# BUTSpeechFIT/x-vector-kaldi-tf

Hardware: AMD Instinct MI355X
Metric: utterances/sec (= x-vectors/sec, 512-d) on synthetic 23-dim MFCC, T~U[200,400] (higher is better)
Workload: dtype f32 in/out, f32 accumulate; GEMM products as fp16 MFMA + 2^-11 x scaled bf8 MFMA of the cross terms (layers 1-4) and bf16x3 split MFMA (layer 0, FC)

## Files before the change

include/xvector_hip.h:

```cpp
#ifndef XVECTOR_HIP_H_
#define XVECTOR_HIP_H_

#include <stddef.h>
#include <stdint.h>

#ifdef __cplusplus
extern "C" {
#endif

#define XV_ACT_NONE 0
#define XV_ACT_RELU 1
#define XV_ACT_LRELU 2
#define XV_ACT_PRELU 3

#define XV_ERR_BAD_ARG (-1)
#define XV_ERR_UNSUPPORTED (-2)

int xv_version(void);
const char *xv_last_error(void);
#define XV_TUNE_TILE_ROWS 1
#define XV_TUNE_FIRST_TILES 2
#define XV_TUNE_FP32_GEMM 3
int xv_set_tuning(int key, int value);

int xv_pack_weights_f32(const float *w, int kred, int cout, float *wp, void *stream);

int xv_fold_bn_f32(const float *gamma, const float *beta, const float *mean, const float *var, float eps,
                   int c, float *scale, float *shift, void *stream);

int xv_fold_shift_taps_f32(const float *w, const float *shift, const float *bias, int K, int cin, int cout, float *tap_bias,
                           float *bias_full, void *stream);

int xv_tdnn_layer_f32(const float *x, int64_t R, int cin, int ldx, const float *wp, const float *bias,
                      const float *bn_scale, const float *bn_shift, int act_kind, const float *act_alpha,
                      int K, int dilation, int cout, const uint8_t *row_valid, float *y, int ldy,
                      float *y_preact, void *stream);

size_t xv_packed_weights_rows_f32_floats(int K, int cin, int ldx, int cout);
int xv_pack_weights_rows_f32(const float *w, int K, int cin, int ldx, int cout, float *wp, void *stream);
int xv_tdnn_layer_rows_f32(const float *x, int64_t R, int cin, int ldx, const float *wp, const float *bias, const float *bn_scale,
                           const float *bn_shift, int act_kind, const float *act_alpha, int K, int cout, const uint8_t *row_valid,
                           float *y, int ldy, void *stream);

int xv_toom_supported(int K, int dilation, int cin, int cout);
size_t xv_packed_weights_toom_f32_floats(int K, int cin, int cout);
int xv_pack_weights_toom_f32(const float *w, int K, int cin, int cout, float *wp, void *stream);
int xv_tdnn_layer_toom_f32(const float *x, int64_t R, int cin, int ldx, const float *wp, const float *bias, const float *bn_scale,
                           const float *bn_shift, int act_kind, const float *act_alpha, int K, int cout, const uint8_t *row_valid,
                           float *y, int ldy, void *stream);
int xv_tdnn_layer_toom_dilated_f32(const float *x, int64_t R, int cin, int ldx, const float *wp, const float *bias, const float *bn_scale,
                                   const float *bn_shift, int act_kind, const float *act_alpha, int K, int dilation, int cout,
                                   const uint8_t *row_valid, float *y, int ldy, void *stream);

#define XV_FMT_F32 0
#define XV_FMT_SPLIT 1
#define XV_SPLIT_PAD_BEFORE 8
#define XV_SPLIT_PAD_AFTER 264
size_t xv_packed_weights_bf16x3_bytes(int K, int cin, int cout);
int xv_pack_weights_bf16x3(const float *w, int K, int cin, int cout, void *wt, void *stream);
int xv_pack_weights_bf16x3_many(int n, const float *const *w, const int32_t *K, const int32_t *cin, const int32_t *cin_pad,
                                const int32_t *cout, void *const *wt_fwd, void *const *wt_bwd, void *stream);
size_t xv_split_row_bytes(int channels);
int xv_split_encode_f32(const float *x, int64_t R, int c, int ldx, void *xs, void *stream);
int xv_split_decode_f32(const void *xs, int64_t R, int c, float *x, int ldx, void *stream);
int xv_tdnn_layer_bf16x3(const void *x, int x_format, int64_t R, int cin, int ldx, const void *wt, const float *bias,
                         const float *bn_scale, const float *bn_shift, int act_kind, const float *act_alpha, int K, int dilation,
                         int cout, const uint8_t *row_valid, void *y, int y_format, int ldy, float *y_preact, int ldpre,
                         void *stream);
int xv_tdnn_layer_bf16x3_sums(const void *x, int x_format, int64_t R, int cin, int ldx, const void *wt, const float *bias,
                              const float *bn_scale, const float *bn_shift, int act_kind, const float *act_alpha, int K,
                              int dilation, int cout, const uint8_t *row_valid, float *y, int ldy, const float *sum_r,
                              int ld_sum_r, void *workspace, void *stream);
int xv_tdnn_layer_bf16x3_moments(const void *x, int x_format, int64_t R, int cin, int ldx, const void *wt, const float *bias,
                                 const float *bn_scale, const float *bn_shift, int act_kind, const float *act_alpha, int K,
                                 int dilation, int cout, const uint8_t *row_valid, float *y, int ldy, float *y_preact, int ldpre,
                                 void *workspace, void *stream);
size_t xv_block_stats_bytes(int64_t R, int cout);
int xv_tdnn_layer_pool_bf16x3(const void *x, int x_format, int64_t R, int cin, int ldx, const void *wt, const float *bias,
                              const float *bn_scale, const float *bn_shift, int act_kind, const float *act_alpha, int K,
                              int dilation, int cout, const uint8_t *row_valid, float *block_stats, void *stream);
int xv_stats_pool_blocks_f32(const float *block_stats, int c, const int32_t *row_start, const int32_t *row_len, int nchunks,
                             float eps, float *out, void *stream);
int xv_tdnn_layer_pool_f32(const float *x, int64_t R, int cin, int ldx, const float *wp, const float *bias, const float *bn_scale,
                           const float *bn_shift, int act_kind, const float *act_alpha, int K, int dilation, int cout,
                           const uint8_t *row_valid, float *block_stats, void *stream);

size_t xv_packed_first_bf16x3_bytes(int K, int cin, int cout);
int xv_pack_first_bf16x3(const float *w, int K, int cin, int cout, void *wt, void *stream);
int xv_tdnn_first_bf16x3(const float *x, int64_t R, int cin, int ldx, const void *wt, const float *bias, const float *bn_scale,
                         const float *bn_shift, int act_kind, const float *act_alpha, int K, int dilation, int cout,
                         const uint8_t *row_valid, void *y, void *stream);

size_t xv_packed_pair_bf16x3_bytes(int cin, int cmid, int cout);
int xv_pack_pair_bf16x3(const float *w1, const float *w2, int cin, int cmid, int cout, void *wt, void *stream);
int xv_tdnn_pair_pool_bf16x3(const void *x, int64_t R, int cin, int cmid, int cout, const void *wt, const float *bias1,
                             const float *bn_scale1, const float *bn_shift1, const float *act_alpha1, const float *bias2,
                             const float *bn_scale2, const float *bn_shift2, const float *act_alpha2, int act_kind,
                             const uint8_t *row_valid, float *block_stats, void *stream);

#define XV_FMT_SPLIT8 2
size_t xv_packed_weights_f16bf8_bytes(int K, int cin, int cout);
int xv_pack_weights_f16bf8(const float *w, int K, int cin, int cout, void *wt, void *stream);
int xv_split8_encode_f32(const float *x, int64_t R, int c, int ldx, void *xs, int32_t *status, void *stream);
int xv_split8_decode_f32(const void *xs, int64_t R, int c, float *x, int ldx, void *stream);
int xv_tdnn_layer_f16bf8(const void *x, int64_t R, int cin, const void *wt, const float *bias, const float *bn_scale,
                         const float *bn_shift, int act_kind, const float *act_alpha, int K, int dilation, int cout,
                         const uint8_t *row_valid, const float *tap_bias, void *y, int y_format, int ldy, int32_t *status,
                         void *stream);
int xv_tdnn_layer_pool_f16bf8(const void *x, int64_t R, int cin, const void *wt, const float *bias, const float *bn_scale,
                              const float *bn_shift, int act_kind, const float *act_alpha, int K, int dilation, int cout,
                              const uint8_t *row_valid, const float *tap_bias, float *block_stats, void *stream);
int xv_tdnn_first_f16bf8(const float *x, int64_t R, int cin, int ldx, const void *wt, const float *bias, const float *bn_scale,
                         const float *bn_shift, int act_kind, const float *act_alpha, int K, int dilation, int cout,
                         const uint8_t *row_valid, void *y, int32_t *status, void *stream);

size_t xv_packed_pair_f16bf8_bytes(int cin, int cmid, int cout);
int xv_pack_pair_f16bf8(const float *w1, const float *w2, int cin, int cmid, int cout, void *wt, void *stream);
int xv_tdnn_pair_pool_f16bf8(const void *x, int64_t R, int cin, int cmid, int cout, const void *wt, const float *bias1,
                             const float *bn_scale1, const float *bn_shift1, const float *act_alpha1, const float *bias2,
                             const float *bn_scale2, const float *bn_shift2, const float *act_alpha2, int act_kind,
                             const uint8_t *row_valid, float *block_stats, int32_t *status, void *stream);

size_t xv_packed_pair_f16mx6_bytes(int cin, int cmid, int cout);
int xv_pack_pair_f16mx6(const float *w1, const float *w2, int cin, int cmid, int cout, void *wt, void *stream);
int xv_tdnn_pair_pool_f16mx6(const void *x, int64_t R, int cin, int cmid, int cout, const void *wt, const float *bias1,
                             const float *bn_scale1, const float *bn_shift1, const float *act_alpha1, const float *bias2,
                             const float *bn_scale2, const float *bn_shift2, const float *act_alpha2, int act_kind,
                             const uint8_t *row_valid, float *block_stats, int32_t *status, void *stream);

#define XV_FMT_SPLIT6 3
size_t xv_packed_weights_f16mx6_bytes(int K, int cin, int cout);
int xv_pack_weights_f16mx6(const float *w, int K, int cin, int cout, void *wt, void *stream);
int xv_split6_encode_f32(const float *x, int64_t R, int c, int ldx, void *xs, int32_t *status, void *stream);
int xv_split6_decode_f32(const void *xs, int64_t R, int c, float *x, float *cq, int ldx, void *stream);
int xv_tdnn_layer_f16mx6(const void *x, int64_t R, int cin, const void *wt, const float *bias, const float *bn_scale,
                         const float *bn_shift, int act_kind, const float *act_alpha, int K, int dilation, int cout,
                         const uint8_t *row_valid, const float *tap_bias, void *y, int y_format, int ldy, int32_t *status,
                         void *stream);

int xv_fc_bf16x3(const float *x, int nrows, int in_dim, const void *wt, const float *bias, const float *bn_scale,
                 const float *bn_shift, int act_kind, const float *act_alpha, int out_dim, float *y, float *y_preact, void *stream);

size_t xv_stats_pool_workspace_bytes(int c, int nchunks, int max_len, int split_rows);
int xv_stats_pool_f32(const float *h, int64_t ldh, int c, const int32_t *row_start, const int32_t *row_len,
                      int nchunks, int max_len, int split_rows, float eps, float *out, void *workspace,
                      void *stream);

int xv_fc_f32(const float *x, int nrows, int in_dim, const float *wp, const float *bias, const float *bn_scale,
              const float *bn_shift, int act_kind, const float *act_alpha, int out_dim, float *y,
              float *y_preact, void *stream);

size_t xv_fc_splitk_workspace_bytes(int nrows, int in_dim, int out_dim);
int xv_fc_splitk_f32(const float *x, int nrows, int in_dim, const float *wp, const float *bias, const float *bn_scale,
                     const float *bn_shift, int act_kind, const float *act_alpha, int out_dim, float *y, float *y_preact, void *workspace,
                     void *stream);

int xv_chunk_average_f32(const float *e, const int32_t *seg_start, const int32_t *chunk_len, int nutts, int dim,
                         float *out, void *stream);


int xv_chunk_moments_f32(const float *h, int64_t ldh, int c, const int32_t *row_start, const int32_t *row_len, int nchunks,
                         int max_len, int split_rows, float *out, void *workspace, void *stream);
int xv_merge_moments_f32(const float *chunk_mean_var, const int32_t *row_len, int nchunks, int c, float *mean, float *var,
                         void *stream);
int xv_rows_affine_f32(const float *x, int ldx, int64_t R, int c, const float *scale, const float *shift,
                       const uint8_t *row_valid, float *y, int ldy, void *stream);
int xv_rows_affine_split_f32(const float *x, int ldx, int64_t R, int c, const float *scale, const float *shift,
                             const uint8_t *row_valid, float *y, int ldy, void *y_split, void *stream);
size_t xv_wgrad_workspace_bytes(int64_t R, int cin, int cout, int K);
int xv_wgrad_f32(const float *x, int ldx, const float *dz, int lddz, int64_t R, int cin, int cout, int K, int dilation,
                 float *dw, void *workspace, void *stream);
int xv_wgrad_bf16x3(const float *x, int ldx, const float *dz, int lddz, int64_t R, int cin, int cout, int K, int dilation,
                    float *dw, void *workspace, void *stream);
size_t xv_wgrad_bias_workspace_bytes(int64_t R, int cin, int cout, int K);
int xv_wgrad_bias_bf16x3(const float *x, int ldx, const float *dz, int lddz, int64_t R, int cin, int cout, int K, int dilation,
                         float *dw, float *db, void *workspace, void *stream);
size_t xv_col_sums_workspace_bytes(int64_t R, int c);
int xv_col_sums_f32(const float *a, int lda, const float *b, int ldb, int64_t R, int c, float *sum_a, float *sum_ab,
                    void *workspace, void *stream);
int xv_bn_act_backward_f32(const float *dh, const float *r, int ld, int64_t R, int c, const float *sum_dh,
                           const float *sum_dh_r, const float *mean, const float *var, const float *gamma, float eps,
                           float n_frames, int act_kind, float act_alpha, const uint8_t *row_valid, float *dgamma,
                           float *dbeta, float *coef_ws, float *dz, void *stream);
int xv_bn_act_backward_split_f32(const float *dh, const float *r, int ld, int64_t R, int c, const float *sum_dh,
                                 const float *sum_dh_r, const float *mean, const float *var, const float *gamma, float eps,
                                 float n_frames, int act_kind, float act_alpha, const uint8_t *row_valid, float *dgamma,
                                 float *dbeta, float *coef_ws, float *dz, void *dz_split, void *stream);
int xv_bn_act_backward_parts_f32(const float *dh, const float *r, int ld, int64_t R, int c, const void *sums_workspace,
                                 const float *mean, const float *var, const float *gamma, float eps, float n_frames,
                                 int act_kind, float act_alpha, const uint8_t *row_valid, float *dgamma, float *dbeta,
                                 float *coef_ws, float *dz, void *dz_split, void *stream);
int xv_bn_moments_fold_f32(const void *sums_workspace, int64_t R, int c, float n_frames, const float *gamma, const float *beta,
                           float eps, float *mean, float *var, float *scale, float *shift, void *stream);
int xv_col_sums_merge_f32(const void *sums_workspace, int64_t R, int c, float *sum_a, float *sum_ab, void *stream);
int xv_pool_bn_act_backward_f32(const float *h, const float *r, int ld, int c, const int32_t *row_start, const int32_t *row_len,
                                int nchunks, int64_t R, const float *pooled, const float *dpooled, const float *chunk_moments,
                                const float *mean, const float *var, const float *gamma, float eps, float n_frames,
                                int act_kind, float act_alpha, float *dgamma, float *dbeta, float *coef_ws, float *dz,
                                void *dz_split, void *stream);
int xv_bn_small_forward_f32(const float *x, int ldx, int nrows, int c, const float *gamma, const float *beta, float eps, float *mean,
                            float *var, float *y, int ldy, void *stream);
int xv_bn_small_backward_f32(const float *dh, const float *r, int ld, int nrows, int c, const float *mean, const float *var,
                             const float *gamma, float eps, int act_kind, float act_alpha, float *dgamma, float *dbeta, float *dz,
                             void *stream);
int xv_pool_backward_f32(const float *h, int ldh, int c, const int32_t *row_start, const int32_t *row_len, int nchunks,
                         int64_t R, const float *pooled, const float *dpooled, float *dh, void *stream);
int xv_softmax_ce_f32(const float *logits, const int32_t *labels, int nrows, int nclasses, float *loss_acc, float *row_ws,
                      float *dlogits, void *stream);
int xv_adam_f32(float *param, const float *grad, float *m, float *v, int64_t n, float lr_t, float beta1, float beta2, float eps,
                void *stream);
int xv_axpy_f32(float *y, const float *x, float a, int64_t n, void *stream);
size_t xv_sumsq_workspace_bytes(int64_t n);
int xv_sumsq_f32(const float *x, int64_t n, float *out, void *workspace, void *stream);
int xv_dropout_f32(float *x, int ldx, int64_t R, int c, uint64_t seed, float keep_prob, void *stream);
int xv_minibatch_layout(int B, int T, int gap, int64_t rows, int32_t *row_start, int32_t *row_len, uint8_t *row_valid, void *stream);
int xv_pack_minibatch_f32(const void *src, int src_is_f16, int B, int T, int F, int gap, int in_dim, float *dst, int64_t rows,
                          void *stream);

int xv_prelu_backward_f32(float *dr, float *z, int ld, int64_t R, int c, const float *alpha, void *stream);

int xv_ema_f32(float *moving, const float *batch, int n, float decay, void *stream);

int xv_l2_normalize_rows_f32(const float *x, int ldx, int nrows, int c, float *y, int ldy, float *norm, void *stream);
int xv_l2_normalize_backward_f32(const float *dy, const float *y, const float *norm, int nrows, int c, float *dx, void *stream);
int xv_am_margin_f32(float *cosines, const int32_t *labels, int nrows, int nclasses, float scale, float margin, void *stream);

int xv_attention_scores_f32(const float *u, int64_t ldu, int64_t R, int c, const float *v, float *scores, float *nonlin,
                            int64_t ldn, void *stream);
int xv_attention_softmax_f32(const float *scores, const int32_t *row_start, const int32_t *row_len, int nchunks, float *att,
                             void *stream);
size_t xv_attention_pool_workspace_bytes(int c, int nchunks, int max_len, int split_rows);
int xv_attention_pool_f32(const float *h, int64_t ldh, int c, const float *att, const int32_t *row_start, const int32_t *row_len,
                          int nchunks, int max_len, int split_rows, float eps, float *out, void *workspace, void *stream);
int xv_attention_pool_backward_f32(const float *h, int64_t ldh, int c, const float *att, const int32_t *row_start,
                                   const int32_t *row_len, int nchunks, int max_len, const float *pooled, const float *dpooled,
                                   float *dh, int64_t lddh, float *datt, void *stream);
int xv_attention_softmax_backward_f32(const float *att, const float *datt, const int32_t *row_start, const int32_t *row_len,
                                      int nchunks, float *dscores, void *stream);
int xv_attention_scores_backward_f32(float *nonlin, int64_t ldn, const float *dscores, const float *v, int64_t R, int c, float *du,
                                     int64_t lddu, void *stream);

int xv_cmn_sliding_scatter_f32(const float *x, int ldx, int feat_dim, const int32_t *utt_start, const int32_t *utt_len,
                               int n_utts, int max_len, int cmn_window, int center, int min_window, const int32_t *dst_row,
                               float *y, int ldy, void *stream);

#define XV_BACKEND_KSTEP 8
#define XV_SIDE_PLAIN 0
#define XV_SIDE_ENROL 1
#define XV_SIDE_TEST 2
#define XV_SIDE_COSINE 3
int xv_backend_prepare_f32(const float *x, int64_t ldx, int n_rows, int dim_in, const int32_t *num_utts, const float *mean,
                           const float *lda, int64_t ld_lda, const float *lda_offset, int dim, int length_norm,
                           const float *plda_transform, const float *plda_mean, const float *plda_psi, int side, float *out,
                           int64_t ldo, float *r, void *stream);
int xv_score_matrix_f32(const float *e, const float *t, int64_t ldk, int kpad, int n_enrol, int n_test, const float *r,
                        float *scores, int64_t ld_scores, void *stream);
int xv_score_blocks_f32(const float *e, const float *t, int64_t ldk, int kpad, int n_rows, const float *r, const int32_t *grp_row0,
                        const int64_t *grp_score0, int n_groups, int max_n, float *scores, int64_t scores_elems, int32_t *status,
                        void *stream);
int xv_score_pairs_f32(const float *e, const float *t, int64_t ldk, int kpad, const int32_t *e_idx, const int32_t *t_idx,
                       int64_t n_trials, const float *r, float *scores, void *stream);
int xv_topk_row_stats_f32(const float *scores, int64_t ld, int n_rows, int n_cols, int top_n, float *mean, float *std,
                          void *stream);

#define XV_MOMENT_SLAB 2048
int xv_moment_stats_f64(const float *x, int64_t ldx, int64_t n_rows, int dim, double *sum, double *outer, int64_t ld_outer,
                        void *workspace, size_t workspace_bytes, void *stream);
size_t xv_moment_stats_workspace_bytes(int64_t n_rows, int dim);

#define XV_AHC_MAX_N 32768
int xv_ahc_average_f64(const float *scores, int64_t ld, int n, double threshold, int min_clusters, int32_t *merge_a,
                       int32_t *merge_b, double *merge_score, int32_t *n_merges, int32_t *labels, void *workspace,
                       size_t workspace_bytes, void *stream);
size_t xv_ahc_average_workspace_bytes(int n);

#define XV_AHC_BATCH_MAX_N 4096
int xv_ahc_average_batch_f64(const float *scores, int64_t scores_elems, const int32_t *grp_row0, const int64_t *grp_score0,
                             const int64_t *grp_ws0, const double *threshold, const int32_t *min_clusters, int n_groups, int max_n,
                             int n_rows, int32_t *merge_a, int32_t *merge_b, double *merge_score, int32_t *n_merges, int32_t *labels,
                             int32_t *status, void *workspace, size_t workspace_bytes, void *stream);
size_t xv_ahc_average_batch_workspace_bytes(int n);

#define XV_PCA_MAX_DIM 128
#define XV_PCA_MAX_SWEEPS 30
int xv_pca_plda_groups_f64(const float *y, int64_t ldy, int n_rows, const int32_t *grp_row0, int n_groups, int dim,
                           double target_energy, const double *mean, const double *within, const double *between,
                           const double *transform, const double *psi, int32_t *grp_dim, int32_t *grp_info, double *eigvals,
                           double *pca, double *grp_psi, double *grp_map, double *grp_off, int32_t *status, void *workspace,
                           size_t workspace_bytes, void *stream);
size_t xv_pca_plda_groups_workspace_bytes(int n_groups, int dim);
int xv_backend_prepare_groups_f32(const float *y, int64_t ldy, int n_rows, const int32_t *grp_row0, int n_groups, int max_n, int dim,
// ... 118 lines not shown
```

x-vector-kaldi-tf_amd/csrc/xv_first.hip:

```cpp
#include "xv_device.h"
#include "xv_split8.h"

namespace {

std::atomic<int> g_first_tiles{0};

constexpr int FR_WAVES = 8;
constexpr int FR_TILES = 3;
constexpr int FR_NKS = 4;
constexpr int FR_PASS_COLS = 128;
constexpr int FR_W_BYTES = (FR_PASS_COLS / 16) * FR_NKS * 2048;
constexpr int FR_P_OFF = 2 * FR_W_BYTES;
constexpr int FR_MAX_COUT = 512;
constexpr size_t FR_LDS_BYTES = FR_P_OFF + 4 * FR_MAX_COUT * 4;
constexpr int SROW = 128;
static_assert(FR_TILES == 3, "tdnn_first_kernel dispatches first_block<.., 1 | 2 | 3>");

struct FirstParams {
    const float *x;
    long R;
    int ldx, kc;
    int K, dil, cout;
    const uint8_t *wt;
    const float *bias, *scale, *shift, *alpha;
    int act;
    const uint8_t *valid;
    uint8_t *y;
    int ychunks;
    long row_base, rows_here;
    long n_tiles;
    int tpw;
    int *status;
};

template <int MODE>
__device__ __forceinline__ float first_act(float z, float a)
{
    if constexpr (MODE == 2) return __builtin_bit_cast(float, max(__builtin_bit_cast(int, z), 0));
    return MODE == 1 ? fmaxf(a * z, z) : MODE == 2 ? fmaxf(z, 0.f) : fmaxf(z, 0.f) + a * fminf(z, 0.f);
}

template <int HALF>
__device__ __forceinline__ float sub_f16_half(float c, int hpair)
{
    float r;
    if constexpr (HALF == 0)
        asm("v_fma_mix_f32 %0, %1, -1.0, %2 op_sel:[0,0,0] op_sel_hi:[1,0,0]" : "=v"(r) : "v"(hpair), "v"(c));
    else
        asm("v_fma_mix_f32 %0, %1, -1.0, %2 op_sel:[1,0,0] op_sel_hi:[1,0,0]" : "=v"(r) : "v"(hpair), "v"(c));
    return r;
}

constexpr int FR_STORE_AUX = 2;

template <int MODE, bool Y8, int NT, bool MASK, bool CLAMP>
__device__ __forceinline__ void first_block(const bf16x8 (&xh)[FR_TILES][FR_NKS], const bf16x8 (&xl)[FR_TILES][FR_NKS],
                                            const bf16x8 (&wh0)[FR_NKS], const bf16x8 (&wl0)[FR_NKS], const bf16x8 (&wh1)[FR_NKS],
                                            const bf16x8 (&wl1)[FR_NKS], const f32x4 b0, const f32x4 b1, const f32x4 s0, const f32x4 s1,
                                            const f32x4 o0, const f32x4 o1, const f32x4 a0, const f32x4 a1, const int (&keepm)[FR_TILES],
                                            const unsigned (&hioff)[FR_TILES], const int slab_off, const __amdgpu_buffer_rsrc_t yrs,
                                            float &amax)
{
    f32x4 m0[NT], m1[NT];
    auto mfma_tile = [&](int j) {
        m0[j] = b0; m1[j] = b1;
#pragma unroll
        for (int u = 0; u < FR_NKS; ++u) {
            m0[j] = __builtin_amdgcn_mfma_f32_16x16x32_bf16(wl0[u], xh[j][u], m0[j], 0, 0, 0);
            m1[j] = __builtin_amdgcn_mfma_f32_16x16x32_bf16(wl1[u], xh[j][u], m1[j], 0, 0, 0);
            m0[j] = __builtin_amdgcn_mfma_f32_16x16x32_bf16(wh0[u], xl[j][u], m0[j], 0, 0, 0);
            m1[j] = __builtin_amdgcn_mfma_f32_16x16x32_bf16(wh1[u], xl[j][u], m1[j], 0, 0, 0);
            m0[j] = __builtin_amdgcn_mfma_f32_16x16x32_bf16(wh0[u], xh[j][u], m0[j], 0, 0, 0);
            m1[j] = __builtin_amdgcn_mfma_f32_16x16x32_bf16(wh1[u], xh[j][u], m1[j], 0, 0, 0);
        }
    };
    auto epilogue = [&](int j) {
        const f32x4 z0 = m0[j], z1 = m1[j];
        float v[8];
#pragma unroll
        for (int e = 0; e < 4; e += 2) {
            const f32x2 r0 = {first_act<MODE>(z0[e], a0[e]), first_act<MODE>(z0[e + 1], a0[e + 1])};
            const f32x2 r1 = {first_act<MODE>(z1[e], a1[e]), first_act<MODE>(z1[e + 1], a1[e + 1])};
            const f32x2 y0 = __builtin_elementwise_fma(r0, (f32x2){s0[e], s0[e + 1]}, (f32x2){o0[e], o0[e + 1]});
            const f32x2 y1 = __builtin_elementwise_fma(r1, (f32x2){s1[e], s1[e + 1]}, (f32x2){o1[e], o1[e + 1]});
            v[e] = y0[0]; v[e + 1] = y0[1]; v[4 + e] = y1[0]; v[5 + e] = y1[1];
        }
        if constexpr (Y8) {
            typedef _Float16 f16x2 __attribute__((ext_vector_type(2)));
            typedef short s16x2 __attribute__((ext_vector_type(2)));
            xv_i32x4 vh, vx;
            float lo[8];
#pragma unroll
            for (int i = 0; i < 8; i += 2) {
                amax = fmaxf(amax, fmaxf(fabsf(v[i]), fabsf(v[i + 1])));
                float ca = v[i], cb = v[i + 1];
                if constexpr (CLAMP) {
                    ca = __builtin_amdgcn_fmed3f(ca, -XV_SPLIT8_MAX, XV_SPLIT8_MAX);
                    cb = __builtin_amdgcn_fmed3f(cb, -XV_SPLIT8_MAX, XV_SPLIT8_MAX);
                }
                if constexpr (MASK) {
                    ca = __builtin_bit_cast(float, __builtin_bit_cast(int, ca) & keepm[j]);
                    cb = __builtin_bit_cast(float, __builtin_bit_cast(int, cb) & keepm[j]);
                }
                const f16x2 h = {(_Float16)ca, (_Float16)cb};
                vh[i >> 1] = __builtin_bit_cast(int, h);
                lo[i] = sub_f16_half<0>(ca, vh[i >> 1]);
                lo[i + 1] = sub_f16_half<1>(cb, vh[i >> 1]);
                v[i] = ca; v[i + 1] = cb;
            }
            constexpr float inv = 1.f / XV_SPLIT8_LO_SCALE;
            s16x2 t0 = {0, 0}, t1 = {0, 0};
            t0 = __builtin_amdgcn_cvt_scalef32_pk_bf8_f32(t0, lo[0], lo[1], inv, false);
            t0 = __builtin_amdgcn_cvt_scalef32_pk_bf8_f32(t0, lo[2], lo[3], inv, true);
            t1 = __builtin_amdgcn_cvt_scalef32_pk_bf8_f32(t1, lo[4], lo[5], inv, false);
            t1 = __builtin_amdgcn_cvt_scalef32_pk_bf8_f32(t1, lo[6], lo[7], inv, true);
            int h0 = __builtin_amdgcn_cvt_pk_bf8_f32(v[0], v[1], 0, false);
            h0 = __builtin_amdgcn_cvt_pk_bf8_f32(v[2], v[3], h0, true);
            int h1 = __builtin_amdgcn_cvt_pk_bf8_f32(v[4], v[5], 0, false);
            h1 = __builtin_amdgcn_cvt_pk_bf8_f32(v[6], v[7], h1, true);
            vx = (xv_i32x4){__builtin_bit_cast(int, t0), __builtin_bit_cast(int, t1), h0, h1};
            __builtin_amdgcn_raw_buffer_store_b128(vh, yrs, hioff[j], slab_off, FR_STORE_AUX);
            __builtin_amdgcn_raw_buffer_store_b128(vx, yrs, hioff[j] ^ 64u, slab_off, FR_STORE_AUX);
        } else {
            bf16x8 vh, vl;
#pragma unroll
            for (int e = 0; e < 8; ++e) {
                const float m = MASK ? __builtin_bit_cast(float, __builtin_bit_cast(int, v[e]) & keepm[j]) : v[e];
                const __bf16 h = (__bf16)m;
                vh[e] = h;
                vl[e] = (__bf16)(m - (float)h);
            }
            __builtin_amdgcn_raw_buffer_store_b128(__builtin_bit_cast(xv_i32x4, vh), yrs, hioff[j], slab_off, FR_STORE_AUX);
            __builtin_amdgcn_raw_buffer_store_b128(__builtin_bit_cast(xv_i32x4, vl), yrs, hioff[j] ^ 64u, slab_off, FR_STORE_AUX);
        }
    };
    mfma_tile(0);
    __builtin_amdgcn_sched_barrier(0);
#pragma unroll
    for (int j = 1; j < NT; ++j) {
        mfma_tile(j);
        epilogue(j - 1);
        __builtin_amdgcn_sched_barrier(0);
    }
    epilogue(NT - 1);
    __builtin_amdgcn_sched_barrier(0);
}

template <int MODE, bool Y8>
__global__ __launch_bounds__(FR_WAVES * 64) void tdnn_first_kernel(const FirstParams p)
{
    extern __shared__ __attribute__((aligned(16))) char lds[];
    const int tid = threadIdx.x;
    const int lane = tid & 63;
    const int wave = __builtin_amdgcn_readfirstlane(tid >> 6);
    const int G = lane >> 4, f = lane & 15;
    const long tile0 = ((long)blockIdx.x * FR_WAVES + wave) * p.tpw;
    const int left = ((p.K - 1) * p.dil) >> 1;
    const int n_pass = (p.cout + FR_PASS_COLS - 1) / FR_PASS_COLS;
    const int n_groups = (p.tpw + FR_TILES - 1) / FR_TILES;
    const int steps = n_groups * n_pass;
    const unsigned yrow = (unsigned)p.ychunks * SROW;
    const __amdgpu_buffer_rsrc_t yrs = __builtin_amdgcn_make_buffer_rsrc(p.y + (size_t)p.row_base * yrow, 0, (int)(unsigned)(p.rows_here * yrow), XV_RSRC_FLAGS);

    auto fetch_weights = [&](int ps, int buf) {
        const int pieces = (min(FR_PASS_COLS, p.cout - ps * FR_PASS_COLS) >> 5) * 2 * FR_NKS * 2;
        const uint8_t *src = p.wt + (size_t)ps * FR_W_BYTES + lane * 16;
        char *dst = lds + buf * FR_W_BYTES;
        for (int pc = wave; pc < pieces; pc += FR_WAVES) XV_GLDS16_OFF(src + (size_t)pc * 1024, dst + pc * 1024, 0);
    };
    const int rot = (int)(blockIdx.x % (unsigned)n_pass);
    fetch_weights(rot, 0);
    {
        float *P = reinterpret_cast<float *>(lds + FR_P_OFF);
        for (int c = tid; c < p.cout; c += FR_WAVES * 64) {
            P[c] = p.bias ? p.bias[c] : 0.f;
            P[FR_MAX_COUT + c] = p.scale ? p.scale[c] : 1.f;
            P[2 * FR_MAX_COUT + c] = p.shift ? p.shift[c] : 0.f;
            P[3 * FR_MAX_COUT + c] = p.act == XV_ACT_NONE ? 1.f : p.act == XV_ACT_LRELU ? p.alpha[0] : p.act == XV_ACT_PRELU ? p.alpha[c] : 0.f;
        }
    }
    const f32x4 *P4 = reinterpret_cast<const f32x4 *>(lds + FR_P_OFF);

    bf16x8 xh[FR_TILES][FR_NKS], xl[FR_TILES][FR_NKS];
    int keepm[FR_TILES];
    unsigned hioff[FR_TILES];
    bool group_masked = false, clamping = false;
    int n_live = 0;
    float amax = 0.f;
    int pass = rot, group = 0, in_group = 0;
    int stores_behind_fetch = -1;

    for (int s = 0; s < steps; ++s) {
        if (in_group == 0) {
            const long gtile = tile0 + (long)group * FR_TILES;
            const long lrow0 = gtile * 16;
            n_live = 0;
#pragma unroll
            for (int j = 0; j < FR_TILES; ++j) {
                const bool ex = group * FR_TILES + j < p.tpw && gtile + j < p.n_tiles;
                n_live += ex ? 1 : 0;
                const long lrow = lrow0 + 16 * j + f, row = p.row_base + lrow;
                const bool in = ex && lrow < p.rows_here;
                keepm[j] = (in && (!p.valid || p.valid[row])) ? -1 : 0;
                hioff[j] = in ? (unsigned)lrow * yrow + (unsigned)((G ^ ((int)(row >> 1) & 7)) << 4) : 0x80000000u;
            }
#pragma unroll
            for (int u = 0; u < FR_NKS; ++u) {
                const int k = 32 * u + 8 * G;
                const int tap = k / p.kc;
                const bool live = tap < p.K;
                const int tap_off = tap * p.dil - left;
                const int c0 = k - tap * p.kc;
#pragma unroll
                for (int j = 0; j < FR_TILES; ++j) {
                    const long r = p.row_base + lrow0 + 16 * j + f + tap_off;
                    f32x4 a = {0.f, 0.f, 0.f, 0.f}, b = a;
                    if (live && j < n_live && r >= 0 && r < p.R) {
                        const float *src = p.x + (size_t)r * p.ldx + c0;
                        a = *reinterpret_cast<const f32x4 *>(src);
                        b = *reinterpret_cast<const f32x4 *>(src + 4);
                    }
#pragma unroll
                    for (int e = 0; e < 4; ++e) {
                        const __bf16 ha = (__bf16)a[e], hb = (__bf16)b[e];
                        xh[j][u][e] = ha; xh[j][u][4 + e] = hb;
                        xl[j][u][e] = (__bf16)(a[e] - (float)ha); xl[j][u][4 + e] = (__bf16)(b[e] - (float)hb);
                    }
                }
            }
            group_masked = __builtin_amdgcn_ballot_w64(keepm[0] == 0 || keepm[1] == 0 || keepm[2] == 0) != 0;
            stores_behind_fetch = -1;
        }
        if (stores_behind_fetch == 2 * 4 * FR_TILES) asm volatile("s_waitcnt vmcnt(24)" ::: "memory");
        else if (stores_behind_fetch == 2 * 4 * (FR_TILES - 1)) asm volatile("s_waitcnt vmcnt(16)" ::: "memory");
        else asm volatile("s_waitcnt vmcnt(0)" ::: "memory");
        __syncthreads();
        const int n_pairs = min(FR_PASS_COLS, p.cout - pass * FR_PASS_COLS) >> 5;
        if (s + 1 < steps) fetch_weights(pass + 1 == n_pass ? 0 : pass + 1, (s + 1) & 1);
        stores_behind_fetch = 0;
        const char *wbuf = lds + (s & 1) * FR_W_BYTES + lane * 16;

        if (n_live > 0) {
            for (int t = 0; t < n_pairs; ++t) {
                const int tp = (t + wave) % n_pairs;
                bf16x8 wh0[FR_NKS], wl0[FR_NKS], wh1[FR_NKS], wl1[FR_NKS];
                const char *w0 = wbuf + (size_t)(tp * 2) * (FR_NKS * 2048);
#pragma unroll
                for (int u = 0; u < FR_NKS; ++u) {
                    wh0[u] = *reinterpret_cast<const bf16x8 *>(w0 + u * 2048);
                    wl0[u] = *reinterpret_cast<const bf16x8 *>(w0 + u * 2048 + 1024);
                    wh1[u] = *reinterpret_cast<const bf16x8 *>(w0 + FR_NKS * 2048 + u * 2048);
                    wl1[u] = *reinterpret_cast<const bf16x8 *>(w0 + FR_NKS * 2048 + u * 2048 + 1024);
                }
                const int cb = pass * FR_PASS_COLS + tp * 32 + 8 * G;
                const int c4 = cb >> 2;
                const f32x4 b0 = P4[c4], b1 = P4[c4 + 1], s0 = P4[FR_MAX_COUT / 4 + c4], s1 = P4[FR_MAX_COUT / 4 + c4 + 1],
                            o0 = P4[2 * FR_MAX_COUT / 4 + c4], o1 = P4[2 * FR_MAX_COUT / 4 + c4 + 1];
                f32x4 a0 = {0.f, 0.f, 0.f, 0.f}, a1 = a0;
                if constexpr (MODE != 2) { a0 = P4[3 * FR_MAX_COUT / 4 + c4]; a1 = P4[3 * FR_MAX_COUT / 4 + c4 + 1]; }
                const int slab_off = (pass * (FR_PASS_COLS / 32) + tp) * SROW;
                auto run = [&](auto nt, auto mask, auto clamp) {
                    first_block<MODE, Y8, decltype(nt)::value, decltype(mask)::value, decltype(clamp)::value>(
                        xh, xl, wh0, wl0, wh1, wl1, b0, b1, s0, s1, o0, o1, a0, a1, keepm, hioff, slab_off, yrs, amax);
                };
                auto run_nt = [&](auto mask, auto clamp) {
                    if (n_live == 3) run(std::integral_constant<int, 3>{}, mask, clamp);
                    else if (n_live == 2) run(std::integral_constant<int, 2>{}, mask, clamp);
                    else run(std::integral_constant<int, 1>{}, mask, clamp);
                };
                if (Y8 && clamping) run_nt(std::true_type{}, std::true_type{});
                else {
                    if (group_masked) run_nt(std::true_type{}, std::false_type{});
                    else run_nt(std::false_type{}, std::false_type{});
                    if (Y8 && __builtin_amdgcn_ballot_w64(!(amax <= XV_SPLIT8_MAX)) != 0) {
                        clamping = true;
                        run_nt(std::true_type{}, std::true_type{});
                        stores_behind_fetch = -1000;
                    }
                }
                stores_behind_fetch += 2 * n_live;
            }
        }
        if (++pass == n_pass) pass = 0;
        if (++in_group == n_pass) { in_group = 0; ++group; }
    }
    if constexpr (Y8)
        if (amax > XV_SPLIT8_MAX && p.status) atomicOr(p.status, 1);
}

__global__ void pack_first_kernel(const float *__restrict__ w, int K, int cin, int kc, int cout, uint8_t *__restrict__ wt, size_t total)
{
    const size_t i = (size_t)blockIdx.x * blockDim.x + threadIdx.x;
    if (i >= total) return;
    const int e = (int)(i & 7);
    const int lane = (int)((i >> 3) & 63);
    constexpr int TILES = FR_PASS_COLS / 16;
    const int u = (int)((i >> 9) & 3);
    const int tile = (int)((i >> 11) & (TILES - 1));
    const int pass = (int)(i / (size_t)(512 * FR_NKS * TILES));
    const int k = 32 * u + 8 * (lane >> 4) + e;
    const int tap = k / kc, c = k - tap * kc;
    const int i_row = lane & 15;
    const int col = pass * FR_PASS_COLS + 32 * (tile >> 1) + 8 * (i_row >> 2) + 4 * (tile & 1) + (i_row & 3);
    const float x = (tap < K && c < cin && col < cout) ? w[((size_t)tap * cin + c) * cout + col] : 0.f;
    const __bf16 hi = (__bf16)x;
    const __bf16 lo = (__bf16)(x - (float)hi);
    uint8_t *t = wt + (size_t)pass * FR_W_BYTES + (size_t)(tile * FR_NKS + u) * 2048 + lane * 16 + e * 2;
    *reinterpret_cast<uint16_t *>(t) = __builtin_bit_cast(uint16_t, hi);
    *reinterpret_cast<uint16_t *>(t + 1024) = __builtin_bit_cast(uint16_t, lo);
}

bool first_shape_ok(int K, int cin, int cout)
{
    const int kc = (cin + 7) / 8 * 8;
    return K > 0 && (K & 1) && cin > 0 && K * kc <= 32 * FR_NKS && cout > 0 && (cout & 31) == 0 && cout <= FR_MAX_COUT;
}

}

extern "C" {

void xv_internal_first_tiles(int tiles) { g_first_tiles.store(tiles, std::memory_order_relaxed); }

size_t xv_packed_first_bf16x3_bytes(int K, int cin, int cout)
{
    if (!first_shape_ok(K, cin, cout)) return 0;
    return (size_t)((cout + FR_PASS_COLS - 1) / FR_PASS_COLS) * FR_W_BYTES;
}

int xv_pack_first_bf16x3(const float *w, int K, int cin, int cout, void *wt, void *stream)
{
    if (!w || !wt) return fail(XV_ERR_BAD_ARG, "pack_first_bf16x3: NULL pointer");
    if (!first_shape_ok(K, cin, cout))
        return fail(XV_ERR_UNSUPPORTED, "pack_first_bf16x3: needs K odd, K*ceil8(cin) <= 128, cout % 32 == 0, cout <= 512");
    const size_t total = xv_packed_first_bf16x3_bytes(K, cin, cout) / 4;
    hipLaunchKernelGGL(pack_first_kernel, dim3((unsigned)((total + 255) / 256)), dim3(256), 0, (hipStream_t)stream, w, K, cin,
                       (cin + 7) / 8 * 8, cout, (uint8_t *)wt, total);
    return launch_status();
}

static int first_launch(const float *x, int64_t R, int cin, int ldx, const void *wt, const float *bias, const float *bn_scale,
                        const float *bn_shift, int act_kind, const float *act_alpha, int K, int dilation, int cout,
                        const uint8_t *row_valid, void *y, bool y8, int32_t *status, void *stream)
{
    if (R <= 0) return 0;
    if (!x || !wt || !y) return fail(XV_ERR_BAD_ARG, "tdnn_first: NULL pointer");
    if (act_kind < XV_ACT_NONE || act_kind > XV_ACT_PRELU) return fail(XV_ERR_BAD_ARG, "tdnn_first: unknown act_kind");
    if ((act_kind == XV_ACT_LRELU || act_kind == XV_ACT_PRELU) && !act_alpha) return fail(XV_ERR_BAD_ARG, "tdnn_first: act_alpha is NULL");
    const int kc = (cin + 7) / 8 * 8;
    if (!first_shape_ok(K, cin, cout) || dilation <= 0 || (K - 1) * dilation > 8)
        return fail(XV_ERR_UNSUPPORTED, "tdnn_first: needs K odd, K*ceil8(cin) <= 128, (K-1)*dilation <= 8, cout % 32 == 0, cout <= 512");
    if (ldx < kc || (ldx & 7) || (((uintptr_t)x) & 31))
        return fail(XV_ERR_UNSUPPORTED, "tdnn_first: rows must hold ceil8(cin) floats (padding columns zero), ldx % 8 == 0, x 32-byte aligned");
    if ((((uintptr_t)wt) | ((uintptr_t)y)) & 15) return fail(XV_ERR_BAD_ARG, "tdnn_first: wt and y must be 16-byte aligned");
    FirstParams p{};
    p.x = x; p.R = (long)R; p.ldx = ldx; p.kc = kc; p.K = K; p.dil = dilation; p.cout = cout; p.wt = (const uint8_t *)wt;
    p.bias = bias; p.scale = bn_scale; p.shift = bn_shift; p.alpha = act_alpha; p.act = act_kind; p.valid = row_valid;
    p.y = (uint8_t *)y; p.ychunks = cout / 32; p.status = (int *)status;
    typedef void (*kern_t)(const FirstParams);
    const kern_t kerns[6] = {tdnn_first_kernel<0, false>, tdnn_first_kernel<1, false>, tdnn_first_kernel<2, false>,
                             tdnn_first_kernel<0, true>,  tdnn_first_kernel<1, true>,  tdnn_first_kernel<2, true>};
    static std::atomic<unsigned long long> lds_done{0};
    if (const int rc = opt_in_dynamic_lds(lds_done, kerns, FR_LDS_BYTES)) return rc;
    const int mode = act_kind == XV_ACT_LRELU ? 1 : act_kind == XV_ACT_RELU ? 2 : 0;
    static std::atomic<int> n_cu{0};
    int cus = n_cu.load(std::memory_order_relaxed);
    if (cus <= 0) {
        int dev = 0;
        (void)hipGetDevice(&dev);
        if (hipDeviceGetAttribute(&cus, hipDeviceAttributeMultiprocessorCount, dev) != hipSuccess || cus <= 0) cus = 256;
        n_cu.store(cus, std::memory_order_relaxed);
    }
    const int forced = g_first_tiles.load(std::memory_order_relaxed);
    const long waves = (long)cus * FR_WAVES;
    constexpr long MAX_ROWS = 1L << 19;
    for (long r0 = 0; r0 < p.R; r0 += MAX_ROWS) {
        p.row_base = r0;
        p.rows_here = p.R - r0 < MAX_ROWS ? p.R - r0 : MAX_ROWS;
        p.n_tiles = (p.rows_here + 15) / 16;
        p.tpw = forced > 0 ? forced : (int)((p.n_tiles + waves - 1) / waves);
        const long per_wg = (long)p.tpw * FR_WAVES;
        hipLaunchKernelGGL(kerns[mode + (y8 ? 3 : 0)], dim3((unsigned)((p.n_tiles + per_wg - 1) / per_wg)), dim3(FR_WAVES * 64), FR_LDS_BYTES,
                           (hipStream_t)stream, p);
    }
    return launch_status();
}

int xv_tdnn_first_bf16x3(const float *x, int64_t R, int cin, int ldx, const void *wt, const float *bias, const float *bn_scale,
                         const float *bn_shift, int act_kind, const float *act_alpha, int K, int dilation, int cout,
                         const uint8_t *row_valid, void *y, void *stream)
{
    return first_launch(x, R, cin, ldx, wt, bias, bn_scale, bn_shift, act_kind, act_alpha, K, dilation, cout, row_valid, y, false,
                        nullptr, stream);
}

int xv_tdnn_first_f16bf8(const float *x, int64_t R, int cin, int ldx, const void *wt, const float *bias, const float *bn_scale,
                         const float *bn_shift, int act_kind, const float *act_alpha, int K, int dilation, int cout,
                         const uint8_t *row_valid, void *y, int32_t *status, void *stream)
{
    return first_launch(x, R, cin, ldx, wt, bias, bn_scale, bn_shift, act_kind, act_alpha, K, dilation, cout, row_valid, y, true,
                        status, stream);
}

}
```

x-vector-kaldi-tf_amd/csrc/xv_kernels.hip:

```cpp
#include "xv_device.h"

namespace {

thread_local char g_err[256] = "";

constexpr int BM = 128;
constexpr int BN = 128;
constexpr int BK = 32;
constexpr int LDS_LD = 36;
constexpr int A_ROWS = BM + MAX_SPAN;
constexpr int NT = 256;

struct GemmParams {
    const float *x;
    long R;
    int cin, ldx;
    const float *wp;
    int kred;
    const float *bias, *scale, *shift;
    int act;
    const float *alpha;
    int K, dil, cout;
    const uint8_t *valid;
    float *y;
// ... 610 lines not shown
        X.b0 = *reinterpret_cast<const f32x4 *>(glds + bb);
        X.b1 = *reinterpret_cast<const f32x4 *>(glds + bb + 32 * G_SROW);
    };
    auto mma = [&](const Fr &X) {
#pragma unroll
        for (int j = 0; j < 4; ++j) {
            acc00 = __builtin_amdgcn_mfma_f32_32x32x2f32(X.a0[j], X.b0[j], acc00, 0, 0, 0);
            acc01 = __builtin_amdgcn_mfma_f32_32x32x2f32(X.a0[j], X.b1[j], acc01, 0, 0, 0);
            acc10 = __builtin_amdgcn_mfma_f32_32x32x2f32(X.a1[j], X.b0[j], acc10, 0, 0, 0);
            acc11 = __builtin_amdgcn_mfma_f32_32x32x2f32(X.a1[j], X.b1[j], acc11, 0, 0, 0);
        }
    };
    auto pin = [&]() {
#pragma unroll
        for (int i = 0; i < 4; ++i) {
            __builtin_amdgcn_sched_group_barrier(0x008, 1, 0);
            __builtin_amdgcn_sched_group_barrier(0x100, 1, 0);
        }
        __builtin_amdgcn_sched_group_barrier(0x008, 12, 0);
        __builtin_amdgcn_sched_barrier(0);
    };
    Fr F, G;
    load(F, 0, 0);
    for (int s = 0; s < n_stages; ++s) {
        load(G, s & 1, 1);
        mma(F);
        pin();
        asm volatile("s_waitcnt vmcnt(0) lgkmcnt(0)" ::: "memory");
        __builtin_amdgcn_s_barrier();
        dma(s + 2, s & 1);
        __builtin_amdgcn_sched_barrier(0);
        load(F, (s + 1) & 1, 0);
        mma(G);
        pin();
    }
    asm volatile("s_waitcnt vmcnt(0)" ::: "memory");
    __syncthreads();
    switch (p.act) {
    case XV_ACT_RELU: k1_epilogue<XV_ACT_RELU>(p, glds, Ms, m0, n0, wr, wc, tid, acc00, acc01, acc10, acc11); break;
    case XV_ACT_LRELU: k1_epilogue<XV_ACT_LRELU>(p, glds, Ms, m0, n0, wr, wc, tid, acc00, acc01, acc10, acc11); break;
    case XV_ACT_PRELU: k1_epilogue<XV_ACT_PRELU>(p, glds, Ms, m0, n0, wr, wc, tid, acc00, acc01, acc10, acc11); break;
    default: k1_epilogue<XV_ACT_NONE>(p, glds, Ms, m0, n0, wr, wc, tid, acc00, acc01, acc10, acc11); break;
    }
}

std::atomic<int> g_fp32_form{0};

int launch_gemm(const GemmParams &p0, hipStream_t st)
{
    GemmParams p = p0;
    if (p.R <= 0 || p.cout <= 0) return 0;
    if (p.cin <= 0 || p.K <= 0 || (p.K & 1) == 0 || p.dil <= 0) return fail(XV_ERR_BAD_ARG, "tdnn: K must be odd, dims > 0");
    if ((p.K - 1) * p.dil > MAX_SPAN) return fail(XV_ERR_UNSUPPORTED, "tdnn: (K-1)*dilation > 8 unsupported");
    if ((p.lead == 0 && p.ldx < p.cin) || p.ldy < p.cout) return fail(XV_ERR_BAD_ARG, "tdnn: leading dimension too small");
    if ((p.act == XV_ACT_LRELU || p.act == XV_ACT_PRELU) && !p.alpha) return fail(XV_ERR_BAD_ARG, "tdnn: act_alpha is NULL");
    p.kred = p.K * p.cin;
    p.n_nt = (p.cout + BN - 1) / BN;
    const bool small = ((p.R + BM - 1) / BM) * p.n_nt < 768;
    const int bmt = small ? 64 : BM;
    p.n_mt = (int)((p.R + bmt - 1) / bmt);
    const bool vec = (p.cin % 4 == 0) && (p.ldx % 4 == 0) && (((uintptr_t)p.x) % 16 == 0) && (((uintptr_t)p.wp) % 16 == 0);
    if (p.lead && (!vec || p.K != 1 || p.ypre)) return fail(XV_ERR_UNSUPPORTED, "tdnn_rows: needs 16-byte aligned rows of a multiple of 4 floats");
    const uintptr_t out_bits = (uintptr_t)p.y | (uintptr_t)p.ypre | (uintptr_t)p.bias | (uintptr_t)p.scale | (uintptr_t)p.shift |
                               (p.act == XV_ACT_PRELU ? (uintptr_t)p.alpha : 0);
    p.vec_out = (p.cout % 4 == 0) && (p.ldy % 4 == 0) && (out_bits % 16 == 0);
    if (p.blk && !p.vec_out) return fail(XV_ERR_UNSUPPORTED, "tdnn_pool: needs cout % 4 == 0 and 16-byte aligned per-column parameters");
    typedef void (*kern_t)(const GemmParams);
    const kern_t all[] = {tdnn_gemm_kernel<true, 128>, tdnn_gemm_kernel<false, 128>, tdnn_gemm_kernel<true, 64>,
                          tdnn_gemm_kernel<false, 64>};
    const kern_t dma_all[] = {tdnn_gemm_dma_kernel<1>, tdnn_gemm_dma_kernel<3>, tdnn_gemm_dma_kernel<5>, tdnn_gemm_dma_kernel<7>};
    typedef std::pair<kern_t, size_t> kern_lds;
    const kern_lds lds[] = {{all[0], GEMM_LDS_BYTES}, {all[1], GEMM_LDS_BYTES}, {all[2], GEMM_LDS_BYTES}, {all[3], GEMM_LDS_BYTES},
                            {dma_all[0], F_LDS_BYTES}, {dma_all[1], F_LDS_BYTES}, {dma_all[2], F_LDS_BYTES}, {dma_all[3], F_LDS_BYTES},
                            {tdnn_gemm_k1_kernel, G_LDS_BYTES}};
    static std::atomic<unsigned long long> lds_done{0};
    if (const int rc = opt_in_dynamic_lds(lds_done, lds, [](const kern_lds &kl) { return kl; })) return rc;
    const dim3 grid((unsigned)(p.n_mt * p.n_nt));
    const int form = g_fp32_form.load(std::memory_order_relaxed);
    const bool dma_on = form != 1;
    const bool k1_on = form == 0 || form == 3;
    const bool dma_ok = dma_on && !small && p.k_splits <= 1 && vec && p.vec_out && (p.cin % BK) == 0 && (p.K == 1 || p.K == 3 || p.K == 5 || p.K == 7) &&
                        (p.R + BM + MAX_SPAN) * (long)p.ldx * 4 < (1l << 31) && (long)(p.cout + BN) * p.kred * 4 < (1l << 31);
    if (dma_ok && k1_on && p.K == 1 && p.cin >= 2 * G_BK) {
        hipLaunchKernelGGL(tdnn_gemm_k1_kernel, grid, dim3(NT), G_LDS_BYTES, st, p);
        return launch_status("tdnn_gemm_k1_kernel launch");
    }
    if (dma_ok) {
        const kern_t dk = p.K == 1 ? tdnn_gemm_dma_kernel<1> : p.K == 3 ? tdnn_gemm_dma_kernel<3> : p.K == 5 ? tdnn_gemm_dma_kernel<5>
                                                                                                             : tdnn_gemm_dma_kernel<7>;
        hipLaunchKernelGGL(dk, grid, dim3(NT), F_LDS_BYTES, st, p);
        return launch_status("tdnn_gemm_dma_kernel launch");
    }
    if (p.k_splits > 1) {
        hipLaunchKernelGGL(all[(small ? 2 : 0) + (vec ? 0 : 1)], dim3((unsigned)(p.n_mt * p.n_nt * p.k_splits)), dim3(NT), GEMM_LDS_BYTES, st, p);
        return launch_status("tdnn_gemm_kernel (split-K) launch");
    }
    hipLaunchKernelGGL(all[(small ? 2 : 0) + (vec ? 0 : 1)], grid, dim3(NT), GEMM_LDS_BYTES, st, p);
    return launch_status("tdnn_gemm_kernel launch");
}

__global__ void pack_weights_kernel(const float *__restrict__ w, int kred, int cout, float *__restrict__ wp)
{
    const size_t i = (size_t)blockIdx.x * blockDim.x + threadIdx.x;
    if (i >= (size_t)kred * cout) return;
    const int n = (int)(i / kred), k = (int)(i - (size_t)n * kred);
    wp[i] = w[(size_t)k * cout + n];
}

__global__ void pack_weights_rows_kernel(const float *__restrict__ w, int K, int cin, int ldx, int cout, int kpad, float *__restrict__ wp)
{
    const size_t i = (size_t)blockIdx.x * blockDim.x + threadIdx.x;
    if (i >= (size_t)kpad * cout) return;
    const int o = (int)(i / kpad), col = (int)(i - (size_t)o * kpad);
    const int k = col / ldx, c = col - k * ldx;
    wp[i] = (k < K && c < cin) ? w[((size_t)k * cin + c) * cout + o] : 0.f;
}

__global__ void fold_bn_kernel(const float *gamma, const float *beta, const float *mean, const float *var, float eps,
                               int c, float *scale, float *shift)
{
#pragma clang fp contract(off)
    const int i = blockIdx.x * blockDim.x + threadIdx.x;
    if (i >= c) return;
    const float s = gamma[i] * (1.0f / sqrtf(var[i] + eps));
    float ms = mean[i] * s;
    asm volatile("" : "+v"(ms));
    scale[i] = s;
    shift[i] = beta[i] - ms;
}

__global__ void fold_shift_taps_kernel(const float *__restrict__ w, const float *__restrict__ shift, const float *__restrict__ bias,
                                       int K, int cin, int cout, float *__restrict__ tap, float *__restrict__ bias_full)
{
    const int o = blockIdx.x * blockDim.x + threadIdx.x;
    if (o >= cout) return;
    double total = bias ? (double)bias[o] : 0.0;
    for (int t = 0; t < K; ++t) {
        double acc = 0.0;
        for (int c = 0; c < cin; ++c) acc += (double)shift[c] * (double)w[((size_t)t * cin + c) * cout + o];
        if (tap) tap[(size_t)t * cout + o] = (float)acc;
        total += acc;
    }
    bias_full[o] = (float)total;
}

}

extern "C" {

void xv_internal_gemm3_tile_rows(int value);
void xv_internal_gemm8_tile_rows(int value);
void xv_internal_first_tiles(int tiles);

int xv_version(void) { return 42; }

int xv_set_tuning(int key, int value)
{
    switch (key) {
    case XV_TUNE_TILE_ROWS:
        if (value != 0 && value != 128 && value != 256 && value != 512 && value != 1024)
            return fail(XV_ERR_BAD_ARG, "xv_set_tuning: tile rows must be 0, 128, 256, 512 or 1024");
        xv_internal_gemm3_tile_rows(value >= 512 ? 256 : value);
        xv_internal_gemm8_tile_rows(value);
        return 0;
    case XV_TUNE_FIRST_TILES:
        if (value < 0 || value > 4096) return fail(XV_ERR_BAD_ARG, "xv_set_tuning: first-layer tiles per wave must be 0 .. 4096");
        xv_internal_first_tiles(value);
        return 0;
    case XV_TUNE_FP32_GEMM:
        if (value < 0 || value > 3) return fail(XV_ERR_BAD_ARG, "xv_set_tuning: fp32 GEMM form must be 0, 1, 2 or 3");
        g_fp32_form.store(value, std::memory_order_relaxed);
        return 0;
    default:
        return fail(XV_ERR_BAD_ARG, "xv_set_tuning: unknown key");
    }
}

const char *xv_last_error(void) { return g_err; }

int xv_pack_weights_f32(const float *w, int kred, int cout, float *wp, void *stream)
{
    if (!w || !wp || kred <= 0 || cout <= 0) return fail(XV_ERR_BAD_ARG, "pack_weights: bad argument");
    const size_t n = (size_t)kred * cout;
    hipLaunchKernelGGL(pack_weights_kernel, dim3((unsigned)((n + 255) / 256)), dim3(256), 0, (hipStream_t)stream, w, kred, cout, wp);
    return launch_status("pack_weights_kernel");
}

int xv_fold_bn_f32(const float *gamma, const float *beta, const float *mean, const float *var, float eps, int c,
                   float *scale, float *shift, void *stream)
{
    if (!gamma || !beta || !mean || !var || !scale || !shift || c <= 0) return fail(XV_ERR_BAD_ARG, "fold_bn: bad argument");
    hipLaunchKernelGGL(fold_bn_kernel, dim3((c + 255) / 256), dim3(256), 0, (hipStream_t)stream, gamma, beta, mean, var, eps, c, scale, shift);
    return launch_status("fold_bn_kernel");
}

int xv_fold_shift_taps_f32(const float *w, const float *shift, const float *bias, int K, int cin, int cout, float *tap_bias,
                           float *bias_full, void *stream)
{
    if (!w || !shift || !bias_full || K <= 0 || cin <= 0 || cout <= 0) return fail(XV_ERR_BAD_ARG, "fold_shift_taps: bad argument");
    hipLaunchKernelGGL(fold_shift_taps_kernel, dim3((cout + 63) / 64), dim3(64), 0, (hipStream_t)stream, w, shift, bias, K, cin, cout,
                       tap_bias, bias_full);
    return launch_status("fold_shift_taps_kernel");
}

int xv_tdnn_layer_f32(const float *x, int64_t R, int cin, int ldx, const float *wp, const float *bias,
                      const float *bn_scale, const float *bn_shift, int act_kind, const float *act_alpha, int K,
                      int dilation, int cout, const uint8_t *row_valid, float *y, int ldy, float *y_preact,
                      void *stream)
{
    if (!x || !wp || (!y && !y_preact)) return fail(XV_ERR_BAD_ARG, "tdnn: NULL pointer");
    if (act_kind < XV_ACT_NONE || act_kind > XV_ACT_PRELU) return fail(XV_ERR_BAD_ARG, "tdnn: unknown act_kind");
    GemmParams p{};
    p.x = x; p.R = (long)R; p.cin = cin; p.ldx = ldx; p.wp = wp;
    p.bias = bias; p.scale = bn_scale; p.shift = bn_shift; p.act = act_kind; p.alpha = act_alpha;
    p.K = K; p.dil = dilation; p.cout = cout; p.valid = row_valid; p.y = y; p.ldy = ldy; p.ypre = y_preact;
    return launch_gemm(p, (hipStream_t)stream);
}

size_t xv_packed_weights_rows_f32_floats(int K, int cin, int ldx, int cout)
{
    if (K <= 0 || (K & 1) == 0 || cin <= 0 || ldx < cin || (ldx & 3) || cout <= 0) return 0;
    return (size_t)cout * (((size_t)K * ldx + BK - 1) / BK * BK);
}

int xv_pack_weights_rows_f32(const float *w, int K, int cin, int ldx, int cout, float *wp, void *stream)
{
    const size_t n = xv_packed_weights_rows_f32_floats(K, cin, ldx, cout);
    if (!w || !wp || n == 0) return fail(XV_ERR_BAD_ARG, "pack_weights_rows: K odd, cin <= ldx, ldx % 4 == 0");
    hipLaunchKernelGGL(pack_weights_rows_kernel, dim3((unsigned)((n + 255) / 256)), dim3(256), 0, (hipStream_t)stream, w, K, cin, ldx, cout,
                       (int)(n / cout), wp);
    return launch_status("pack_weights_rows_kernel");
}

int xv_tdnn_layer_rows_f32(const float *x, int64_t R, int cin, int ldx, const float *wp, const float *bias, const float *bn_scale,
                           const float *bn_shift, int act_kind, const float *act_alpha, int K, int cout, const uint8_t *row_valid,
                           float *y, int ldy, void *stream)
{
    if (!x || !wp || !y) return fail(XV_ERR_BAD_ARG, "tdnn_rows: NULL pointer");
    if (act_kind < XV_ACT_NONE || act_kind > XV_ACT_PRELU) return fail(XV_ERR_BAD_ARG, "tdnn_rows: unknown act_kind");
    const size_t n = xv_packed_weights_rows_f32_floats(K, cin, ldx, cout);
    if (n == 0) return fail(XV_ERR_BAD_ARG, "tdnn_rows: K odd, cin <= ldx, ldx % 4 == 0");
    GemmParams p{};
    p.x = x; p.R = (long)R; p.cin = (int)(n / cout); p.ldx = ldx; p.wp = wp;
    p.bias = bias; p.scale = bn_scale; p.shift = bn_shift; p.act = act_kind; p.alpha = act_alpha;
    p.K = 1; p.dil = 1; p.cout = cout; p.valid = row_valid; p.y = y; p.ldy = ldy; p.lead = (K - 1) / 2;
    return launch_gemm(p, (hipStream_t)stream);
}

int xv_tdnn_layer_pool_f32(const float *x, int64_t R, int cin, int ldx, const float *wp, const float *bias, const float *bn_scale,
                           const float *bn_shift, int act_kind, const float *act_alpha, int K, int dilation, int cout,
                           const uint8_t *row_valid, float *block_stats, void *stream)
{
    if (!x || !wp || !block_stats) return fail(XV_ERR_BAD_ARG, "tdnn_pool: NULL pointer");
    if (act_kind < XV_ACT_NONE || act_kind > XV_ACT_PRELU) return fail(XV_ERR_BAD_ARG, "tdnn_pool: unknown act_kind");
    if (((uintptr_t)block_stats) & 15) return fail(XV_ERR_BAD_ARG, "tdnn_pool: block_stats must be 16-byte aligned");
    GemmParams p{};
    p.x = x; p.R = (long)R; p.cin = cin; p.ldx = ldx; p.wp = wp;
    p.bias = bias; p.scale = bn_scale; p.shift = bn_shift; p.act = act_kind; p.alpha = act_alpha;
    p.K = K; p.dil = dilation; p.cout = cout; p.valid = row_valid; p.ldy = cout; p.blk = block_stats;
    return launch_gemm(p, (hipStream_t)stream);
}

int xv_fc_f32(const float *x, int nrows, int in_dim, const float *wp, const float *bias, const float *bn_scale,
              const float *bn_shift, int act_kind, const float *act_alpha, int out_dim, float *y, float *y_preact,
              void *stream)
{
    return xv_tdnn_layer_f32(x, nrows, in_dim, in_dim, wp, bias, bn_scale, bn_shift, act_kind, act_alpha, 1, 1,
                             out_dim, nullptr, y, out_dim, y_preact, stream);
}

static int splitk_groups(int nrows, int in_dim, int out_dim)
{
    if (nrows <= 0 || nrows > 128 || in_dim < 16 * BK) return 1;
    const int chunks = (in_dim + BK - 1) / BK;
    const int tiles = ((nrows + 63) / 64) * ((out_dim + BN - 1) / BN);
    int per = (chunks * tiles + 255) / 256;
    if (per < 2) per = 2;
    return (chunks + per - 1) / per;
}

size_t xv_fc_splitk_workspace_bytes(int nrows, int in_dim, int out_dim)
{
    const int g = splitk_groups(nrows, in_dim, out_dim);
    return g > 1 ? (size_t)g * nrows * out_dim * sizeof(float) : 0;
}

int xv_fc_splitk_f32(const float *x, int nrows, int in_dim, const float *wp, const float *bias, const float *bn_scale,
                     const float *bn_shift, int act_kind, const float *act_alpha, int out_dim, float *y, float *y_preact, void *workspace,
                     void *stream)
{
    const int g = splitk_groups(nrows, in_dim, out_dim);
    if (g <= 1) return xv_fc_f32(x, nrows, in_dim, wp, bias, bn_scale, bn_shift, act_kind, act_alpha, out_dim, y, y_preact, stream);
    if (!x || !wp || (!y && !y_preact) || !workspace) return fail(XV_ERR_BAD_ARG, "fc_splitk: NULL pointer");
    if (act_kind < XV_ACT_NONE || act_kind > XV_ACT_PRELU) return fail(XV_ERR_BAD_ARG, "fc_splitk: unknown act_kind");
    if ((act_kind == XV_ACT_LRELU || act_kind == XV_ACT_PRELU) && !act_alpha) return fail(XV_ERR_BAD_ARG, "fc_splitk: act_alpha is NULL");
    GemmParams p{};
    p.x = x; p.R = nrows; p.cin = in_dim; p.ldx = in_dim; p.wp = wp;
    p.act = XV_ACT_NONE; p.K = 1; p.dil = 1; p.cout = out_dim; p.ldy = out_dim;
    p.ypre = (float *)workspace;
    p.k_splits = g; p.part = (float *)workspace; p.part_stride = (long)nrows * out_dim;
    int rc = launch_gemm(p, (hipStream_t)stream);
    if (rc) return rc;
    const size_t n = (size_t)nrows * out_dim;
    hipLaunchKernelGGL(splitk_reduce_kernel, dim3((unsigned)((n + 255) / 256)), dim3(256), 0, (hipStream_t)stream, (const float *)workspace,
                       (long)nrows * out_dim, g, nrows, out_dim, bias, bn_scale, bn_shift, act_kind, act_alpha, y, out_dim, y_preact, out_dim);
    return launch_status("splitk_reduce_kernel");
}
// ... 5 lines not shown
```

x-vector-kaldi-tf_amd/local/tf/models.py:

```python
import io
import os
import sys
import time

import numpy as np

_PKG_ROOT = os.path.dirname(os.path.dirname(os.path.dirname(os.path.abspath(__file__))))
if _PKG_ROOT not in sys.path:
    sys.path.insert(0, _PKG_ROOT)

import kaldi_io
from xvector_amd import engine, extract_stream, frontend, synthetic, topology, weights as wio

VAR2STD_EPSILON = topology.VAR2STD_EPSILON


def _device():
    dev = os.environ.get("XVECTOR_DEVICE")
    if dev:
        return dev
    return "cuda:%d" % int(os.environ.get("LOCAL_RANK", "0"))


class VectorCollector(object):
# ... 2 lines not shown
    def __init__(self):
        self.keys, self.blocks = [], []

    def write_vectors(self, keys, vecs):
        if len(keys):
            self.keys.extend(keys)
            self.blocks.append(np.asarray(vecs, dtype=np.float32).reshape(len(keys), -1))

    def write(self, data):
        raise IOError("the sharded extractor writes vectors, not bytes")

    def __enter__(self):
        return self

    def __exit__(self, *a):
        return False


def gather_shard_vectors(device_model, collector, shard_keys, rank, world):
    import torch
    from xvector_amd import dist as xdist, jobclock
    dim, dev = device_model.embed_dim, device_model.device
    mine = shard_keys[rank]
    block = np.zeros((len(mine), dim + 1), np.float32)
    if collector.keys:
        whole = len(collector.keys) == len(mine) and mine == collector.keys
        if whole:
            rows = slice(None)
        else:
            rows, j = np.empty(len(collector.keys), np.int64), 0
            for i, k in enumerate(mine):
                if j < len(rows) and collector.keys[j] == k:
                    rows[j] = i
                    j += 1
            if j != len(rows):
                raise RuntimeError("sharded extraction: emitted keys are not a subsequence of the shard's keys")
        block[rows, 0] = 1.0
        if whole and len(collector.blocks) == 1:
            block[:, 1:] = collector.blocks[0]
        else:
            block[rows, 1:] = np.concatenate(collector.blocks)
    xdist.wait_process_group()
    jobclock.mark("wait for the process group")
    import torch.distributed as dist
    host = dist.is_initialized() and dist.get_backend() == "gloo"
    blocks = xdist.gather_blocks(torch.from_numpy(block) if host else torch.from_numpy(block).to(dev), [len(k) for k in shard_keys], 0)
    jobclock.mark("gather")
    if rank != 0:
        return None
    out = []
    for r in range(world):
        got = blocks[r].cpu().numpy()
        out.append((shard_keys[r], got[:, 1:], got[:, 0] > 0.5))
    return out


_SELECTED = {}
_IDLE_MODELS = {}
_IDLE_KEEP = 1


def _checkpoint_identity(model_dir):
    ident = []
    for name in ("model.weights.npz", "model.index", "model.data-00000-of-00001"):
        path = os.path.join(model_dir, name)
        try:
            st = os.stat(path)
            ident.append((os.path.realpath(path), st.st_mtime_ns, st.st_size))
        except OSError:
            pass
    return (tuple(ident) or None,)


class _StepDone(object):

    def __init__(self, value):
        self._value = value

    def result(self):
        return self._value


class Model(object):

    window_frames = 1 << 21
    first_window_frames = 1 << 18
    arena_bytes = 64 << 20
    first_arena_bytes = 64 << 20
    map_input = os.environ.get("XVECTOR_MAP_INPUT", "1") != "0"
    arena_count = 5
    exchange_windows = int(os.environ.get("XVECTOR_EXCHANGE_WINDOWS", "0"))
    max_batch_rows = 262144

    def __init__(self):
        self.graph = None
        self.device_model = None
        self.num_classes = None

    @classmethod
    def class_topology(cls):
        return topology.get(cls.__name__)

    def build_model(self, num_classes, input_feature_dim, output_dir, logger=None):
        if logger is not None:
            logger.info("Start building the model ...")
        topo = self.class_topology()
        self.num_classes = num_classes
        seed = int(os.environ.get("XVECTOR_INIT_SEED", "0"))
        w = synthetic.reference_init(topo, input_feature_dim, num_classes, seed=seed)
        self.save_model(dict(weights=w, topology=topo, model_class=type(self).__name__,
                             num_classes=num_classes, feat_dim=input_feature_dim), output_dir, logger)
        if logger is not None:
            logger.info("Building finished.")

    @staticmethod
    def save_model(sess, output_dir, logger):
        if logger is not None:
            logger.info("Start saving graph ...")
        wio.save_model_dir(output_dir, sess["weights"], sess["topology"], sess["model_class"],
                           sess["num_classes"], sess["feat_dim"])
        if logger is not None:
            logger.info("Graph saved in path: %s" % os.path.join(output_dir, "model"))

    def load_model(self, sess, input_dir, logger):
        if logger is not None:
            logger.info("Start loading graph ...")
        from xvector_amd import jobclock
        w, meta = wio.load_model_dir(input_dir)
        jobclock.once("weights read")
        import torch
        jobclock.once("import torch")
        torch.cuda.init()
        jobclock.once("hip runtime up")
        if getattr(self, "prepin_staging", False):
            try:
                engine.prewarm_staging((int(w["frame_level_info_layer-0/w:0"].shape[1]) + 3) // 4 * 4, self.max_batch_rows)
            except Exception:
                pass
        self.meta = meta
        self.num_classes = meta["num_classes"]
        self.embedding_index = int(os.environ.get("XVECTOR_EMBEDDING_INDEX", "0"))
        self.precision = os.environ.get("XVECTOR_PRECISION", "f16bf8")
        key = _checkpoint_identity(input_dir) + (self.precision, self.embedding_index, _device(), engine.PROBE_LIMIT_F16BF8,
                                                 engine.PROBE_LIMIT_BF16X3, os.environ.get("XVECTOR_ACCURACY_PROBE", "1"))
        known = _SELECTED.get(key)
        idle = _IDLE_MODELS.get(key)
        self._model_key = None
        if known is not None and idle and getattr(self, "_may_borrow", False):
            self.device_model = idle.pop()
            self._model_key = key
        elif known is not None:
            self.device_model = engine.DeviceModel(w, meta["topology"], _device(), self.embedding_index, known["selected"],
                                                   fold_shift=False if known.get("fold_shift") is False else None,
                                                   layer_mx6=False if known.get("layer_mx6") is False else None)
            self.device_model.selection = dict(known, cached=True)
            self._model_key = key
        else:
            self.device_model = engine.select_model(w, meta["topology"], _device(), self.embedding_index, self.precision)
            if key[0] is not None:
                _SELECTED[key] = dict(getattr(self.device_model, "selection", None) or {})
                self._model_key = key
        sel = getattr(self.device_model, "selection", None) or {}
        if logger is not None:
            if sel.get("probed"):
                logger.info("GEMM arithmetic: %s (requested %s; accuracy probe: f16bf8 vs bf16x3 %.2e%s)" % (
                    sel["selected"], sel["requested"], sel["f16bf8_vs_bf16x3"],
                    ", bf16x3 vs fp32 %.2e" % sel["bf16x3_vs_fp32"] if "bf16x3_vs_fp32" in sel else ""))
            logger.info("Graph restored from path: %s" % input_dir)

    def create_one_hot_output_matrix(self, labels):
        one_hot = np.zeros((len(labels), self.num_classes), dtype=np.int32)
        one_hot[np.arange(len(labels)), np.asarray(labels, dtype=np.int64)] = 1
        return one_hot

    def print_models_params(self, input_dir, logger=None):
        w, meta = wio.load_model_dir(input_dir)
        print('\n\nThe components are:\n')
        for name in wio.expected_names(meta["topology"]):
            if name.rsplit('/', 1)[-1] not in ("mean:0", "variance:0"):
                print(name)
        print('\n')

    def get_models_weights(self, input_dir, logger=None):
        h5file = os.path.join(input_dir, 'model.h5')
        try:
            import h5py
        except ImportError:
            h5py = None
        if h5py is not None and os.path.exists(h5file):
            name2weights = {}

            def collect(name, node):
                if not isinstance(node, h5py.Group):
                    name2weights[name] = np.array(node[()])
            with h5py.File(h5file, 'r') as hf:
                hf.visititems(collect)
            return name2weights
        w, meta = wio.load_model_dir(input_dir)
        name2weights = {}
        for name in wio.expected_names(meta["topology"]):
            if name.rsplit('/', 1)[-1] not in ("mean:0", "variance:0"):
                name2weights[name] = np.array(w[name], dtype=np.float32)
        for name in wio.expected_names(meta["topology"]):
            if name not in name2weights:
                name2weights[name] = np.array(w[name], dtype=np.float32)
        for name, mat in name2weights.items():
            print('%s  shape: %s' % (name, str(mat.shape)))
        if h5py is not None:
            with h5py.File(h5file, 'w') as hf:
                for name, mat in name2weights.items():
                    hf.create_dataset(name, data=mat.astype(np.float32))
        elif logger is not None:
            logger.info("h5py is not installed: %s not written" % h5file)
        return name2weights

    def _trainer(self, input_dir, logger, first_batch=None):
        from xvector_amd import trainer
        if logger is not None:
            logger.info("Start loading graph ...")
        w, meta = wio.load_model_dir(input_dir)
        self.meta = meta
        self.num_classes = meta["num_classes"]
        precision = os.environ.get("XVECTOR_TRAIN_PRECISION", "auto")
        adam = wio.load_optimizer_state(input_dir)
        self.train_precision_auto = precision == "auto"
        kept = wio.load_train_verdict(input_dir) if precision == "auto" and first_batch is not None else None
        if kept is not None:
            self.train_precision_verdict = dict(kept, iterations_since_probe=int(kept.get("iterations_since_probe", 0)) + 1, reused=True)
            tr = trainer.Trainer(w, meta["topology"], _device(), adam, precision=kept["selected"])
            if logger is not None:
                logger.info("Training arithmetic: %s (verdict of %d iteration(s) ago, kept with the model)" % (
                    kept["selected"], self.train_precision_verdict["iterations_since_probe"]))
        elif precision == "auto" and first_batch is not None:
            tr, verdict = trainer.select_trainer(w, meta["topology"], _device(), adam, first_batch[0], first_batch[1], logger)
            self.train_precision_verdict = dict(verdict, iterations_since_probe=0)
        else:
            tr = trainer.Trainer(w, meta["topology"], _device(), adam, precision="fp32" if precision == "auto" else precision)
        if logger is not None:
            logger.info("Graph restored from path: %s" % input_dir)
        return tr

    @staticmethod
    def _next_batch(data_loader, index, logger, what, meter):
        import queue
        t0 = time.time()
        try:
            batch, labels = data_loader.pop()
        except queue.Empty:
            logger.warning('Timeout reach when reading %s %d' % (what, index))
            batch, labels = None, None
        else:
            if batch is None:
                logger.warning('batch_data is None for %s %d' % (what, index))
        meter.waited("disk", time.time() - t0)
        return batch, labels

    @staticmethod
    def _everyone_has(batch, device):
        import torch.distributed as dist
        have = batch is not None
        if not (dist.is_available() and dist.is_initialized() and dist.get_world_size() > 1):
            return have
        import torch
        on_gpu = dist.get_backend() == "nccl"
        flag = torch.tensor([1 if have else 0], dtype=torch.int32, device=device if on_gpu else "cpu")
        dist.all_reduce(flag, op=dist.ReduceOp.MIN)
        return bool(flag.item())

    def train_one_iteration(self, data_loader, args, logger):
        from xvector_amd import runstats
        keep_out = float(getattr(args, "dropout_proportion", 0.0) or 0.0)
        seed = int(getattr(args, "random_seed", 0) or 0)
        tr = None
        pending = None
        meter = runstats.Meter(planned=data_loader.count, report_every=args.print_interval)
        for index in range(data_loader.count):
            batch, labels = self._next_batch(data_loader, index, logger, 'the minibatch index', meter)
            stepped_now = self._everyone_has(batch, _device())
            if not stepped_now:
                if batch is not None:
                    logger.warning('minibatch index %d skipped: another rank of the group has no batch' % index)
            else:
                if tr is None:
                    tr = self._trainer(args.input_dir, logger, (batch, labels))
                t0 = time.time()
                launch = getattr(tr, "step_async", None)
                handle = launch(batch, labels, args.learning_rate, keep_out, seed) if launch is not None else \
                    _StepDone(tr.step(batch, labels, args.learning_rate, keep_out, seed))
                now = (index, batch.shape[0], batch.shape[1], handle)
                if pending is not None:
                    meter.stepped(pending[0], pending[1], pending[2], *self._finite(pending, tr, args.input_dir, logger))
                pending = now
                meter.waited("gpu", time.time() - t0)
            if pending is not None and (index == data_loader.count - 1 or meter.interval_due(index)):
                meter.stepped(pending[0], pending[1], pending[2], *self._finite(pending, tr, args.input_dir, logger))
                pending = None
            if not stepped_now:
                meter.skipped(index)
            line = meter.interval_line(index)
            if line:
                logger.info(line)
        for line in meter.training_summary():
            logger.info(line)
        if tr is None:
            tr = self._trainer(args.input_dir, logger)
        if getattr(args, "save_model", True):
            w, adam = tr.export()
# ... 215 lines not shown
```

x-vector-kaldi-tf_amd/xvector_amd/engine.py:

```python
import ctypes
import math
import os
import threading

import numpy as np

from . import hiplib
from . import topology as tp

_HOST = []


def _host_lib():
    if not _HOST:
        lib = None
        path = os.path.join(os.path.dirname(os.path.dirname(os.path.abspath(__file__))), "local", "tf", "libxvector_host.so")
        try:
            if os.environ.get("XVECTOR_NO_HOST_LIB") == "1":
                raise OSError("disabled")
            lib = ctypes.CDLL(path)
            lib.xv_pack_rows_f32.restype = ctypes.c_int
            lib.xv_pack_rows_f32.argtypes = [ctypes.c_void_p, ctypes.c_void_p, ctypes.c_void_p, ctypes.c_int, ctypes.c_int,
                                             ctypes.c_void_p, ctypes.c_int64, ctypes.c_int64, ctypes.c_void_p, ctypes.c_int]
            lib.xv_raw_row_plan.restype = ctypes.c_int
# ... 61 lines not shown
    valid = np.flatnonzero((T > 0) & (T >= min_chunk_size))
    order = valid[np.argsort(T[valid], kind="stable")]
    To = T[order]
    cs = To if chunk_size == -1 else np.where(To < chunk_size, To, chunk_size)
    nch = -(-To // np.maximum(cs, 1))
    last = To - (nch - 1) * cs
    kept = nch - (last < min_chunk_size)
    seg = np.zeros(len(order) + 1, np.int64)
    np.cumsum(kept, out=seg[1:])
    c_utt = np.repeat(order, kept)
    idx = np.arange(int(seg[-1]), dtype=np.int64) - np.repeat(seg[:-1], kept)
    csr = np.repeat(cs, kept)
    c_start = idx * csr
    c_len = np.where(idx == np.repeat(nch - 1, kept), np.repeat(last, kept), csr)
    return order, c_utt, c_start, c_len, seg


def plan_subsegments(num_rows, min_chunk_size, window, period):
    if not 1 <= period <= window:
        raise ValueError("sub-segments need 1 <= period <= window (period %d, window %d)" % (period, window))
    if num_rows == 0 or num_rows < min_chunk_size:
        return None
    plan = [(0, min(window, num_rows))]
    k = 1
    while (k - 1) * period + window < num_rows:
        length = min(window, num_rows - k * period)
        if length < min_chunk_size:
            break
        plan.append((k * period, length))
        k += 1
    return plan


def plan_subsegment_table(lengths, min_chunk_size, window, period):
    if not 1 <= period <= window:
        raise ValueError("sub-segments need 1 <= period <= window (period %d, window %d)" % (period, window))
    T = np.asarray(lengths, dtype=np.int64)
    valid = np.flatnonzero((T > 0) & (T >= min_chunk_size))
    order = valid[np.argsort(T[valid], kind="stable")]
    To = T[order]
    kmax = np.where(To > window, -(-(To - window) // period), 0)
    last = np.minimum(window, To - kmax * period)
    kept = kmax + 1 - ((kmax > 0) & (last < min_chunk_size))
    seg = np.zeros(len(order) + 1, np.int64)
    np.cumsum(kept, out=seg[1:])
    c_utt = np.repeat(order, kept)
    idx = np.arange(int(seg[-1]), dtype=np.int64) - np.repeat(seg[:-1], kept)
    c_start = idx * period
    c_len = np.where(idx == np.repeat(kmax, kept), np.repeat(last, kept), window)
    return order, c_utt, c_start, c_len, seg


def device_plan_table(utt_start, utt_len, order, c_len, seg_start):
    return np.stack([np.asarray(utt_start)[order], np.asarray(utt_len)[order], c_len[seg_start[:-1]], np.diff(seg_start),
                     seg_start[:-1]]).astype(np.int32)


class BatchLayout(object):

    def __init__(self, lengths, gap, align=1):
        lengths = np.asarray(lengths, dtype=np.int64)
        self.gap = int(gap)
        self.align = int(align)
        self.row_len = lengths.astype(np.int32)
        self.lead = int(slot_rows(0, self.gap, self.align))
        self.slots = slot_rows(lengths, self.gap, self.align)
        starts = np.empty(len(lengths), dtype=np.int64)
        if len(lengths):
            starts[0] = self.lead
            np.cumsum(self.slots[:-1], out=starts[1:])
            starts[1:] += self.lead
        self.row_start = starts.astype(np.int32)
        self.rows = int(self.lead + self.slots.sum())
        self.nchunks = len(lengths)
        self.max_len = int(lengths.max()) if len(lengths) else 0
        assert self.rows < 2 ** 31

    def row_valid(self, out=None):
        n = self.nchunks
        vals = np.zeros(2 * n + 1, dtype=np.uint8)
        vals[1::2] = 1
        reps = np.empty(2 * n + 1, dtype=np.int64)
        reps[0] = self.lead
        reps[1::2] = self.row_len
        reps[2::2] = self.slots - self.row_len
        m = np.repeat(vals, reps)
        if out is not None:
            out[:self.rows] = m
            return out[:self.rows]
        return m

    def pack(self, mats, out):
        if not mats:
            out[:self.rows] = 0
            return
        F = mats[0].shape[1]
        z = np.zeros((self.gap + self.align, F), dtype=out.dtype)
        parts = [z[:self.lead]] * (2 * len(mats) + 1)
        parts[1::2] = mats
        if self.align > 1:
            parts[2::2] = [z[:g] for g in (self.slots - self.row_len).tolist()]
        elif self.lead != self.gap:
            raise AssertionError
        np.concatenate(parts, axis=0, out=out[:self.rows, :F])


def shift_tap_table(w3d, shift):
    return np.einsum("c,kco->ko", np.asarray(shift, np.float64), np.asarray(w3d, np.float64))


def folded_row_bias(bias, taps, row_valid, dilation):
    taps = np.asarray(taps, np.float64)
    K = taps.shape[0]
    v = np.asarray(row_valid, np.float64).reshape(-1)
    R = v.shape[0]
    halo = (K - 1) // 2 * int(dilation)
    vp = np.concatenate([np.zeros(halo), v, np.zeros(halo)])
    out = np.tile(np.asarray(bias, np.float64), (R, 1))
    for t in range(K):
        out += vp[t * int(dilation): t * int(dilation) + R, None] * taps[t][None, :]
    return out


class _ColumnView(object):

    def __init__(self, weights, cols):
        self.weights, self.cols = weights, cols

    def __getitem__(self, name):
        return self.weights[name][self.cols]


class _Layer(dict):

    def __missing__(self, key):
        if key == "wp" and "_make_wp" in self:
            self["wp"] = dict.pop(self, "_make_wp")()
            return self["wp"]
        raise KeyError(key)

    def ep(self, act):
        return self["bias"], self["scale"], self["shift"], act, self["alpha"]

    @property
    def pp(self):
        return self["bias"], self["scale"], self["shift"], self["alpha"]


class DeviceModel(object):

    POOL_SPLIT_ROWS = 512

    def __init__(self, weights, topo, device="cuda:0", embedding_index=0, precision="bf16x3", fused_pool=None, pair_kernel=None,
                 first_kernel=None, fold_shift=None, layer_mx6=None):
        import torch
        hiplib.require_gpu()
        assert precision in ("fp32", "fp32tc", "bf16x3", "f16bf8")
        self.toom = precision == "fp32tc"
        self.requested_precision = precision
        if self.toom:
            precision = "fp32"
        self.f16bf8 = False
        if precision == "f16bf8":
            precision = "bf16x3"
            ks, ds = list(topo["kernel_sizes"]), list(topo["dilations"])
            w0 = weights["frame_level_info_layer-0/w:0"]
            self.f16bf8 = (not tp.is_attention(topo) and fused_pool in (None, True) and len(ks) >= 3 and (ks[0] - 1) * ds[0] <= 8 and
                           all(hiplib.f16bf8_supported(k, d) for k, d in zip(ks[1:], ds[1:])))
        self.precision = precision
        self._weights = weights if self.f16bf8 else None
        self._fallback = None
        self.attention = tp.is_attention(topo)
        can_fuse = not self.attention and (precision == "bf16x3" or int(topo["layer_sizes"][-1]) % 4 == 0)
        self.fused_pool = can_fuse if fused_pool is None else bool(fused_pool)
        assert not (self.fused_pool and precision == "fp32" and int(topo["layer_sizes"][-1]) % 4), "fused fp32 pooling needs Cout % 4 == 0"
        assert not (self.fused_pool and self.attention), "the fused epilogue computes plain statistics, not attention-weighted ones"
        self.align = hiplib.POOL_BLOCK_ROWS if self.fused_pool else (2 if self.toom else 1)
        self.torch = torch
        self.device = torch.device(device)
        self.topo = topo
        self.embedding_index = int(embedding_index)
        self.gap = tp.max_halo(topo)
        self.act = tp.ACT_CODES[topo.get("activation", "relu")]
        self.feat_dim = int(weights["frame_level_info_layer-0/w:0"].shape[1])
        self.in_dim = (self.feat_dim + 3) // 4 * 4
        self.layers = []
        self._uploaded = {}
        with torch.cuda.device(self.device):
            for i, (k, d) in enumerate(zip(topo["kernel_sizes"], topo["dilations"])):
                sc = "frame_level_info_layer-%d" % i
                w = weights[sc + "/w:0"]
                assert w.shape[0] == k, "kernel size mismatch in %s" % sc
                if i == 0 and self.in_dim != self.feat_dim:
                    wpad = np.zeros((k, self.in_dim, w.shape[2]), np.float32)
                    wpad[:, :self.feat_dim] = w
                    w = wpad
                last = i == len(topo["kernel_sizes"]) - 1
                self.layers.append(self._prep(weights, sc, w, k, d, defer_wp=self.f16bf8, toom_ok=not (last and self.fused_pool)))
                if isinstance(self.layers[-1].get("wp"), hiplib.PackedToom) and d > 1:
                    self.align = math.lcm(self.align, 2 * int(d))
            if self.attention:
                A = self.layers[-1]["cout"] // 2
                self.att_dim = A
                aw = weights["attention/w:0"]
                assert aw.shape == (A, A), "attention/w:0 must be [%d, %d]" % (A, A)
                self.att = dict(K=1, dil=1, cin=A, cout=A, bias=self._dev(weights["attention/b:0"]),
                                v=self._dev(weights["attention/v:0"]))
                if precision == "bf16x3":
                    self.att["wp"] = hiplib.pack_weights_bf16x3(self._dev(aw[None, :, :]))
                    sc = "frame_level_info_layer-%d" % (len(self.layers) - 1)
                    k, d = topo["kernel_sizes"][-1], topo["dilations"][-1]
                    self.last_halves = [self._prep(weights, sc, weights[sc + "/w:0"], k, d, cols=slice(a, a + A)) for a in (0, A)]
                else:
                    self.att["wp"] = hiplib.pack_weights(self._dev(aw))
            self.first = None
            L0 = self.layers[0]
            if (first_kernel is None or first_kernel) and precision == "bf16x3" and len(self.layers) > 1 and \
                    self.in_dim % 8 == 0 and hiplib.first_supported(L0["K"], self.in_dim, L0["cout"]) and (L0["K"] - 1) * L0["dil"] <= 8:
                w0 = weights["frame_level_info_layer-0/w:0"]
                wpad = np.zeros((L0["K"], self.in_dim, w0.shape[2]), np.float32)
                wpad[:, :self.feat_dim] = w0
                self.first = hiplib.pack_first_bf16x3(self._dev(wpad))
            assert not (first_kernel and self.first is None), "first_kernel=True but the topology / precision does not allow it"
            self.pair = self.pair8 = self.pair_mx6 = None
            if (pair_kernel is None or pair_kernel) and self.fused_pool and precision == "bf16x3" and len(self.layers) >= 3:
                La, Lb = self.layers[-2], self.layers[-1]
                if La["K"] == 1 and Lb["K"] == 1 and hiplib.pair_supported(La["cin"], La["cout"], Lb["cout"]):
                    n = len(self.layers)
                    wa = self._wdev(weights, "frame_level_info_layer-%d/w:0" % (n - 2))[0]
                    wb = self._wdev(weights, "frame_level_info_layer-%d/w:0" % (n - 1))[0]
                    self.pair = hiplib.pack_pair_bf16x3(wa, wb)
                    if self.f16bf8 and hiplib.pair8_supported(La["cin"], La["cout"], Lb["cout"]):
                        self.pair8 = hiplib.pack_pair_f16bf8(wa, wb)
                        if hiplib.pair_mx6_supported(La["cin"], La["cout"], Lb["cout"]):
                            self.pair_mx6 = hiplib.pack_pair_f16mx6(wa, wb)
            assert not (pair_kernel and self.pair is None), "pair_kernel=True but the topology / precision does not allow it"
            if self.f16bf8:
                if self.first is None:
                    self.layers[0]["wp"]
                n = len(self.layers)
                for i in range(1, n - 2 if self.pair is not None else n):
                    sc = "frame_level_info_layer-%d" % i
                    self.layers[i]["wp8"] = hiplib.pack_weights_f16bf8(self._wdev(weights, sc + "/w:0"))
                self.status = torch.zeros(1, dtype=torch.int32, device=self.device)
            self.mx6_layers = set()
            if self.f16bf8 and (layer_mx6 is None or layer_mx6):
                def takes(j):
                    Lj = self.layers[j]
                    return hiplib.layer_mx6_supported(Lj["K"], Lj["dil"], Lj["cin"], Lj["cout"])
                for i in range(2, n - 2 if self.pair is not None else n - 1):
                    if takes(i) and takes(i - 1):
                        self.layers[i]["wp6"] = hiplib.pack_weights_f16mx6(self._wdev(weights, "frame_level_info_layer-%d/w:0" % i))
                        self.mx6_layers.add(i)
            self.layer_mx6 = bool(self.mx6_layers)
            assert not (layer_mx6 and not self.layer_mx6), \
                "layer_mx6=True needs an f16bf8 model with a K in {3,5,7} layer (Cin % 64 == 0, Cout % 256 == 0) behind another one"
            can_fold = self.f16bf8 and self.act == tp.ACT_RELU and all(L["cout"] % 8 == 0 for L in self.layers[1:] if L["K"] > 1)
            self.fold_shift = can_fold and (fold_shift is None or bool(fold_shift))
            assert not (fold_shift and not self.fold_shift), \
                "fold_shift=True needs an f16bf8 model with ReLU whose K > 1 layers behind layer 0 have widths that are multiples of 8"
            if self.fold_shift:
                for i in range(1, len(self.layers)):
                    L = self.layers[i]
                    w = self._wdev(weights, "frame_level_info_layer-%d/w:0" % i)
                    L["tapbias"], L["fbias"] = hiplib.fold_shift_taps(w, self.layers[i - 1]["shift"], L["bias"], table=L["K"] > 1)
            self.embed = []
            for j in range(len(topo["embedding_sizes"])):
                sc = "embed_layer-%d" % j
                self.embed.append(self._prep(weights, sc, weights[sc + "/w:0"][None, :, :], 1, 1))
            torch.cuda.synchronize()
        self._uploaded = {}
        self.pooled_dim = tp.pooled_dim(topo)
        self.embed_dim = self.embed[self.embedding_index]["cout"]
        self._cap_rows = 0
        self._cap_chunks = 0
        self._pool_ws = None
        self._a0 = None

    @property
    def arithmetic(self):
        return "f16bf8" if self.f16bf8 else ("fp32tc" if self.toom else self.precision)

    def probe_vectors(self, batch):
        torch = self.torch
        x, rs, rl, rv, max_len = batch
        with torch.cuda.device(self.device):
            dx, drs, drl, drv = (torch.from_numpy(np.ascontiguousarray(a)).to(self.device) for a in (x, rs, rl, rv))
            out = torch.empty((len(rs), self.embed_dim), dtype=torch.float32, device=self.device)
            if self.f16bf8:
                self.status.zero_()
            self.forward_packed(dx, drs, drl, drv, len(rs), int(max_len), out)
            return out.cpu().numpy()

    def fallback(self):
        if self._fallback is None:
            assert self.f16bf8
            self._fallback = DeviceModel(self._weights, self.topo, self.device, self.embedding_index, "bf16x3")
        return self._fallback

    def _dev(self, a):
        return self.torch.as_tensor(np.array(a, dtype=np.float32, order="C")).to(self.device)

    def _wdev(self, weights, key):
        if key not in self._uploaded:
            self._uploaded[key] = self._dev(weights[key])
        return self._uploaded[key]

    def _prep(self, weights, scope, w3d, k, d, cols=slice(None), defer_wp=False, toom_ok=True):
        w3d = w3d[:, :, cols]
        weights = _ColumnView(weights, cols)
        layer = _Layer(K=k, dil=d, cin=w3d.shape[1], cout=w3d.shape[2])
        if self.precision == "bf16x3":
            make = lambda: hiplib.pack_weights_bf16x3(self._dev(w3d))
        elif self.toom and scope == "frame_level_info_layer-0" and d == 1 and w3d.shape[1] == self.in_dim and \
                w3d.shape[2] % 4 == 0:
            make = lambda: hiplib.pack_weights_rows(self._dev(w3d), self.in_dim)
        elif self.toom and toom_ok and hiplib.toom_supported(k, d, w3d.shape[1], w3d.shape[2]):
            make = lambda: hiplib.pack_weights_toom(self._dev(w3d))
        else:
            make = lambda: hiplib.pack_weights(self._dev(w3d.reshape(-1, w3d.shape[2])))
        if defer_wp:
            layer["_make_wp"] = make
        else:
            layer["wp"] = make()
        layer["bias"] = self._dev(weights[scope + "/b:0"])
        layer["scale"], layer["shift"] = hiplib.fold_bn(*(self._dev(weights["%s/%s:0" % (scope, n)])
                                                          for n in ("gamma", "beta", "mean", "variance")),
                                                        tp.BN_EPSILON)
        layer["alpha"] = None
        if self.act == tp.ACT_LRELU:
            layer["alpha"] = self._dev(np.array([self.topo.get("lrelu_alpha", 0.2)]))
        elif self.act == tp.ACT_PRELU:
            layer["alpha"] = self._dev(weights[scope + "/prelu/prelu:0"])
        return layer

    def reserve(self, rows, nchunks, max_len=None):
        torch = self.torch
        if rows > self._cap_rows:
            self._cap_rows = int(rows)
            widths = sorted(set(l["cout"] for l in self.layers[:-1]))
            wmax = max(widths) if widths else self.layers[-1]["cout"]
            if self.precision == "bf16x3":
                self._ping = hiplib.SplitBuf(self._cap_rows, wmax, self.device)
                self._pong = hiplib.SplitBuf(self._cap_rows, wmax, self.device)
            else:
                self._ping = torch.empty((self._cap_rows, wmax), dtype=torch.float32, device=self.device)
                self._pong = torch.empty((self._cap_rows, wmax), dtype=torch.float32, device=self.device)
            if self.f16bf8 and self.first is None:
                self._l0_rows = torch.empty((self._cap_rows, self.layers[0]["cout"]), dtype=torch.float32, device=self.device)
            if self.fused_pool:
                self._last = torch.empty(hiplib.block_stats_floats(self._cap_rows, self.layers[-1]["cout"]), dtype=torch.float32,
                                         device=self.device)
            elif self.attention:
                A = self.att_dim
                if self.precision == "bf16x3":
                    self._h1 = hiplib.SplitBuf(self._cap_rows, A, self.device)
                    self._last = torch.empty((self._cap_rows, A), dtype=torch.float32, device=self.device)
                else:
                    self._last = torch.empty((self._cap_rows, 2 * A), dtype=torch.float32, device=self.device)
                self._u = torch.empty((self._cap_rows, A), dtype=torch.float32, device=self.device)
                self._scores = torch.empty(self._cap_rows, dtype=torch.float32, device=self.device)
                self._att = torch.zeros(self._cap_rows, dtype=torch.float32, device=self.device)
            else:
                self._last = torch.empty((self._cap_rows, self.layers[-1]["cout"]), dtype=torch.float32, device=self.device)
        if nchunks > self._cap_chunks:
            self._cap_chunks = int(nchunks)
            self._pooled = torch.empty((self._cap_chunks, self.pooled_dim), dtype=torch.float32, device=self.device)
            self._pool_ws = None
        if max_len is not None and not self.fused_pool:
            if self.attention:
                need = hiplib.attention_pool_workspace_bytes(self.att_dim, self._cap_chunks, max_len, self.POOL_SPLIT_ROWS)
            else:
                need = hiplib.stats_pool_workspace_bytes(self.layers[-1]["cout"], self._cap_chunks, max_len, self.POOL_SPLIT_ROWS)
            if need and (self._pool_ws is None or self._pool_ws.numel() * 4 < need):
                self._pool_ws = torch.empty((need + 3) // 4, dtype=torch.float32, device=self.device)

    def _view(self, buf, rows, width):
        if isinstance(buf, hiplib.SplitBuf):
            return buf if buf.channels == width else buf.view(width)
        return buf.view(-1)[: rows * width].view(rows, width)

    def frame_level(self, x, row_start, row_len, row_valid, nchunks, max_len, pooled, events=None, status=None):
        R = x.shape[0]
        self.reserve(R, nchunks, max_len)
        h = x
        bufs = (self._ping, self._pong)
        if events is not None:
            events[0].record()
        layers = self.layers
        if self.f16bf8:
            self._frame_level_f16bf8(x, R, row_valid, self.status if status is None else status)
            layers = ()
        for i, L in enumerate(layers):
            last = i == len(self.layers) - 1
            if i == 0 and self.first is not None and isinstance(bufs[0], hiplib.SplitBuf):
                y = self._view(bufs[0], R, L["cout"])
                hiplib.tdnn_first(h, R, self.first, *L.ep(self.act), L["dil"], row_valid, y)
                h = y
                continue
            if self.pair is not None and i == len(self.layers) - 2:
                hiplib.tdnn_pair_pool(h, R, self.pair, L.pp, self.layers[-1].pp, self.act, row_valid, self._last)
                break
            if last and self.fused_pool:
                hiplib.tdnn_layer_pool(h, R, L["wp"], *L.ep(self.act), L["dil"], row_valid, self._last, K=L["K"])
                break
            if last and self.attention:
                h = self._attention_scores(h, R, L, row_valid)
                break
            y = self._view(self._last if last else bufs[i & 1], R, L["cout"])
            hiplib.tdnn_layer(h, L["wp"], *L.ep(self.act), L["K"], L["dil"], row_valid, y, rows=R)
            h = y
        if events is not None:
            events[1].record()
        if self.fused_pool:
            hiplib.stats_pool_blocks(self._last, self.layers[-1]["cout"], row_start, row_len, nchunks, tp.VAR2STD_EPSILON, pooled)
        elif self.attention:
            hiplib.attention_softmax(self._scores, row_start, row_len, nchunks, self._att)
            hiplib.attention_pool(h, self._att, row_start, row_len, nchunks, max_len, self.POOL_SPLIT_ROWS, tp.VAR2STD_EPSILON,
                                  pooled, self._pool_ws)
        else:
            hiplib.stats_pool(h, row_start, row_len, nchunks, max_len, self.POOL_SPLIT_ROWS, tp.VAR2STD_EPSILON, pooled,
                              self._pool_ws)
        if events is not None:
            events[2].record()
        return pooled

    def _frame_level_f16bf8(self, x, R, row_valid, status, marks=None):
        def mark(label):
            if marks is not None:
                ev = self.torch.cuda.Event(enable_timing=True)
                ev.record()
                marks.append((label, ev))
        n = len(self.layers)
        bufs = (self._ping, self._pong)
        S8, S3, S6 = hiplib.FMT_SPLIT8, hiplib.FMT_SPLIT, hiplib.FMT_SPLIT6
        fold = self.fold_shift

        def pp(i):
            L = self.layers[i]
            if not fold:
                return L.pp
            return L["fbias"] if i else L["bias"], L["scale"], L["shift"] if i == n - 1 else None, L["alpha"]

        def ep(i):
            b, sc, sh, al = pp(i)
            return b, sc, sh, self.act, al

        def taps(i):
            return self.layers[i].get("tapbias") if fold else None
        L = self.layers[0]
        stop = n - 2 if self.pair is not None else n - 1
        pair_fmt = S8 if self.pair8 is not None else S3
        h = bufs[0].view(L["cout"], pair_fmt if (self.pair is not None and stop == 1) else S8)
        mark("start")
        if self.first is not None:
            hiplib.tdnn_first(x, R, self.first, *ep(0), L["dil"], row_valid, h, status)
            mark("layer 0: tdnn_first_kernel (bf16x3)")
        else:
            y32 = self._l0_rows[:R]
            hiplib.tdnn_layer(x, L["wp"], *ep(0), L["K"], L["dil"], row_valid, y32, rows=R)
            hiplib.split_encode(y32, h, rows=R, status=status if h.fmt == S8 else None)
            mark("layer 0: tdnn_gemm_bf16x3_kernel + split encode")
        for i in range(1, stop):
            L = self.layers[i]
            y = bufs[i & 1].view(L["cout"], pair_fmt if (self.pair is not None and i == stop - 1) else
                                 S6 if i + 1 in self.mx6_layers else S8)
            hiplib.tdnn_layer8(h, R, L["wp6" if i in self.mx6_layers else "wp8"], *ep(i), L["dil"], row_valid, y, status, tapbias=taps(i))
            mark("layer %d: tdnn_gemm_f16bf8 (K=%d, %d -> %d)" % (i, L["K"], L["cin"], L["cout"]))
            h = y
        if self.pair is not None:
            pa, pb = pp(n - 2), pp(n - 1)
            if self.pair_mx6 is not None:
                hiplib.tdnn_pair_pool_mx6(h, R, self.pair_mx6, pa, pb, self.act, row_valid, self._last, status)
            elif self.pair8 is not None:
                hiplib.tdnn_pair_pool8(h, R, self.pair8, pa, pb, self.act, row_valid, self._last, status)
            else:
                hiplib.tdnn_pair_pool(h, R, self.pair, pa, pb, self.act, row_valid, self._last)
        else:
            L = self.layers[-1]
            hiplib.tdnn_layer_pool8(h, R, L["wp8"], *ep(n - 1), L["dil"], row_valid, self._last, tapbias=taps(n - 1))
        mark("layers %d+%d + pooling statistics: %s" % (n - 2, n - 1, "tdnn_pair_pool_f16bf8_kernel" if self.pair8 is not None else
                                                        "tdnn_pair_pool_kernel (bf16x3)") if self.pair is not None else
             "layer %d + pooling statistics: tdnn_gemm_f16bf8 POOL" % (n - 1))

    def _attention_scores(self, h, R, L, row_valid):
        A, T = self.att_dim, self.att
        u = self._u[:R]
        if self.precision == "bf16x3":
            L1, L2 = self.last_halves
            hiplib.tdnn_layer(h, L1["wp"], *L1.ep(self.act), L1["K"], L1["dil"], row_valid, self._h1, rows=R)
            h2 = self._last[:R]
            hiplib.tdnn_layer(h, L2["wp"], *L2.ep(self.act), L2["K"], L2["dil"], row_valid, h2, rows=R)
            h1 = self._h1
        else:
            y = self._last[:R]
            hiplib.tdnn_layer(h, L["wp"], *L.ep(self.act), L["K"], L["dil"], row_valid, y, rows=R)
            h1, h2 = y[:, :A], y[:, A:]
        hiplib.tdnn_layer(h1, T["wp"], T["bias"], None, None, tp.ACT_NONE, None, 1, 1, None, u, rows=R)
        hiplib.attention_scores(u, T["v"], self._scores, rows=R)
        return h2

    def segment_level(self, pooled, out):
        n = pooled.shape[0]
        E0 = self.embed[0]
        if self.embedding_index == 0:
            hiplib.fc(pooled, E0["wp"], E0["bias"], None, None, tp.ACT_NONE, None, None, out)
        else:
            if self._a0 is None or self._a0.shape[0] < n:
                self._a0 = self.torch.empty((n, E0["cout"]), dtype=self.torch.float32, device=self.device)
            a0 = self._a0[:n]
            hiplib.fc(pooled, E0["wp"], *E0.ep(self.act), a0, None)
            E1 = self.embed[1]
            hiplib.fc(a0, E1["wp"], E1["bias"], None, None, tp.ACT_NONE, None, None, out)
        return out

    def forward_packed(self, x, row_start, row_len, row_valid, nchunks, max_len, out):
        self.reserve(x.shape[0], nchunks, max_len)
        pooled = self.frame_level(x, row_start, row_len, row_valid, nchunks, max_len, self._pooled[:nchunks])
        return self.segment_level(pooled, out)

    def intermediates_packed(self, x, row_valid):
        torch = self.torch
        R = x.shape[0]
        outs = []
        h = x
        for i, L in enumerate(self.layers):
            last = i == len(self.layers) - 1
            if self.precision == "bf16x3" and not last:
                y = hiplib.SplitBuf(R, L["cout"], self.device)
            else:
                y = torch.empty((R, L["cout"]), dtype=torch.float32, device=self.device)
            hiplib.tdnn_layer(h, L["wp"], *L.ep(self.act), L["K"], L["dil"], row_valid, y, rows=R)
            outs.append(hiplib.split_decode(y, R) if isinstance(y, hiplib.SplitBuf) else y)
            h = y
        return outs


PROBE_LIMIT_F16BF8 = 2e-5
PROBE_LIMIT_BF16X3 = 4e-5
DATA_PROBE_LIMIT = 3e-5
_PROBE_INPUT = {}


def probe_batch(feat_dim, in_dim, gap, align, chunks=8, frames=256, seed=20240917):
    key = (feat_dim, in_dim, gap, align, chunks, frames, seed)
    if key not in _PROBE_INPUT:
        rng = np.random.default_rng(seed)
        rho = 0.92
        t = np.arange(frames)
        L = np.tril(rho ** np.maximum(t[:, None] - t[None, :], 0))
        scale = 12.0 / (1.0 + np.arange(feat_dim)) ** 0.7
        mats = []
        for _ in range(chunks):
            m = L @ (rng.standard_normal((frames, feat_dim)) * np.sqrt(1.0 - rho * rho))
            t0 = int(rng.integers(0, max(frames - 10, 1)))
            m[t0:t0 + 10] *= 4.0
            m *= scale
            mats.append((m - m.mean(axis=0, keepdims=True)).astype(np.float32))
        lay = BatchLayout([frames] * chunks, gap, align)
        x = np.zeros((lay.rows, in_dim), np.float32)
        lay.pack(mats, x)
        _PROBE_INPUT[key] = (x, lay.row_start, lay.row_len, lay.row_valid(), lay.max_len)
    return _PROBE_INPUT[key]


def _max_rel_l2(a, b):
    a, b = np.asarray(a, np.float64), np.asarray(b, np.float64)
    if not (np.isfinite(a).all() and np.isfinite(b).all()):
        return float("inf")
    num = np.sqrt(((a - b) ** 2).sum(axis=1))
    den = np.sqrt((b ** 2).sum(axis=1))
    with np.errstate(invalid="ignore", divide="ignore"):
        r = np.where(den > 0, num / den, np.where(num > 0, np.inf, 0.0))
    return float(np.nan_to_num(r, nan=np.inf).max()) if len(r) else 0.0


def select_model(weights, topo, device="cuda:0", embedding_index=0, precision="f16bf8", probe=None, fold_shift=None, layer_mx6=None):
    if probe is None:
        probe = os.environ.get("XVECTOR_ACCURACY_PROBE", "1") != "0"
    model = DeviceModel(weights, topo, device, embedding_index, precision, fold_shift=fold_shift, layer_mx6=layer_mx6)
    sel = dict(requested=precision, selected=model.arithmetic, probed=False)
    model.selection = sel
    if not probe or not model.f16bf8:
        return model
    batch = probe_batch(model.feat_dim, model.in_dim, model.gap, model.align)
    got = model.probe_vectors(batch)
    clamped = int(model.status.item()) != 0
    model.status.zero_()
    twin = model.fallback()
    ref = twin.probe_vectors(batch)
    err = _max_rel_l2(got, ref)
    sel.update(probed=True, layer_mx6=model.layer_mx6, f16bf8_vs_bf16x3=err, f16bf8_limit=PROBE_LIMIT_F16BF8, probe_left_fp16_range=clamped,
               probe_frames=int(np.sum(batch[2])))
    if err <= PROBE_LIMIT_F16BF8 and not clamped:
        return model
    last, last_err = model, err
    if model.fold_shift and fold_shift is None:
        plain = DeviceModel(weights, topo, device, embedding_index, precision, fold_shift=False, layer_mx6=layer_mx6)
        got = plain.probe_vectors(batch)
        clamped2 = int(plain.status.item()) != 0
        plain.status.zero_()
        err2 = _max_rel_l2(got, ref)
        sel.update(folded_f16bf8_vs_bf16x3=err, f16bf8_vs_bf16x3=err2, probe_left_fp16_range=clamped2, fold_shift=False)
        if err2 <= PROBE_LIMIT_F16BF8 and not clamped2:
            plain._fallback = twin
            plain.selection = sel
            return plain
        last, last_err = plain, err2
    if last.layer_mx6 and layer_mx6 is None:
        bf8 = DeviceModel(weights, topo, device, embedding_index, precision, fold_shift=last.fold_shift, layer_mx6=False)
        got = bf8.probe_vectors(batch)
        clamped3 = int(bf8.status.item()) != 0
        bf8.status.zero_()
        err_bf8 = _max_rel_l2(got, ref)
        sel.update(mx6_f16bf8_vs_bf16x3=last_err, f16bf8_vs_bf16x3=err_bf8, probe_left_fp16_range=clamped3, layer_mx6=False)
        if err_bf8 <= PROBE_LIMIT_F16BF8 and not clamped3:
            bf8._fallback = twin
            bf8.selection = sel
            return bf8
    rung = "fp32" if os.environ.get("XVECTOR_EXACT_RUNG", "fp32tc") == "fp32" else "fp32tc"
    exact = DeviceModel(weights, topo, device, embedding_index, rung)
    err3 = _max_rel_l2(ref, exact.probe_vectors(batch))
    sel.update(bf16x3_vs_fp32=err3, bf16x3_limit=PROBE_LIMIT_BF16X3, exact_rung=exact.arithmetic)
    chosen = twin if err3 <= PROBE_LIMIT_BF16X3 else exact
    sel["selected"] = chosen.arithmetic
    chosen.selection = sel
    return chosen


class _Rows(object):

    def __init__(self, mats, idx, lens, addrs):
        self.mats, self.idx = mats, np.asarray(idx, np.int64)
        self.lengths = np.asarray(lens, np.int64)[self.idx]
        self.addrs = None if addrs is None else np.asarray(addrs, np.uint64)[self.idx]

    def __len__(self):
        return len(self.idx)

    def __getitem__(self, i):
        return self.mats[int(self.idx[i])]

    def __iter__(self):
        for i in self.idx.tolist():
            yield self.mats[i]


_STAGE_CACHE = {}
_STAGE_LOCK = threading.Lock()


_STAGE_PENDING = {}


def _new_stage(torch, in_dim, rows, nchunks, nbuf):
    return [dict(x=torch.zeros((rows, in_dim), dtype=torch.float32).pin_memory(), rv=torch.zeros(rows, dtype=torch.uint8).pin_memory(),
                 meta=torch.zeros((2, nchunks), dtype=torch.int32).pin_memory(), event=None) for _ in range(nbuf)]


def prewarm_staging(in_dim, rows=262144, nchunks=8192):
    import torch
    key = (int(in_dim), Extractor.NBUF)
    with _STAGE_LOCK:
        if key in _STAGE_PENDING or any(st[0]["x"].shape[0] >= rows for st in _STAGE_CACHE.get(key, [])):
            return

        def run():
            try:
                stage = _new_stage(torch, key[0], rows, nchunks, key[1])
                with _STAGE_LOCK:
                    _STAGE_CACHE.setdefault(key, []).append(stage)
            except Exception:
                pass
        th = threading.Thread(target=run, name="xv-pin-staging", daemon=True)
        _STAGE_PENDING[key] = th
    th.start()


def _park_stage(holder):
    if len(holder) == 2 and holder[1] is not None:
        key, stage = holder
        for st in stage:
            if st.get("event") is not None:
                st["event"].synchronize()
                st["event"] = None
        with _STAGE_LOCK:
            parked = _STAGE_CACHE.setdefault(key, [])
            if len(parked) < 2 and all(p is not stage for p in parked):
                parked.append(stage)
        holder[:] = []


class Extractor(object):

    NBUF = 3
    PROBE_ROWS = 16384
    PROBE_EVERY = 64

    def __init__(self, model, min_chunk_size, chunk_size, max_batch_rows=262144, max_batch_chunks=8192, accuracy_probe=None,
                 window=None, period=None):
        self.model = model
        self.window = self.period = None
        if window is not None:
            self.window = int(window)
            self.period = self.window if period is None else int(period)
            if self.period < 1 or self.period > self.window:
                raise ValueError("period must lie in [1, window] (period %d, window %d)" % (self.period, self.window))
            if self.window < int(min_chunk_size):
                raise ValueError("window %d is shorter than min_chunk_size %d" % (self.window, int(min_chunk_size)))
        elif period is not None:
            raise ValueError("period without window")
        if accuracy_probe is None:
            accuracy_probe = os.environ.get("XVECTOR_ACCURACY_PROBE", "1") != "0"
        self.accuracy_probe = bool(accuracy_probe) and model.f16bf8
        self.demoted = False
        self._windows = 0
        self.min_chunk_size = int(min_chunk_size)
        self.chunk_size = int(chunk_size)
        self.max_batch_rows = int(max_batch_rows)
        self.max_batch_chunks = int(max_batch_chunks)
        self.stats = dict(batches=0, chunks=0, frames=0, rows=0)
        self._stage = None
        self._raw_stage = None
        self._plan_stage = None
        self._sub_stage = None
        self._copy_stream = None
        self._turn = 0
        self._finalizer = None
        self._holder = []
        self._pin_free = {}
        self._fallback_ex = None

    def _staging(self, rows, nchunks):
        torch = self.model.torch
        if self._stage is None or self._stage[0]["x"].shape[0] < rows or self._stage[0]["meta"].shape[1] < nchunks:
            rows, nchunks = self._regular_caps(rows, nchunks, self.PIN_FLOOR, self.max_batch_rows)
            if self._stage is not None:
                _park_stage(self._holder)
            with _STAGE_LOCK:
                pending = _STAGE_PENDING.pop((self.model.in_dim, self.NBUF), None)
            if pending is not None:
                pending.join()
            with _STAGE_LOCK:
                parked = _STAGE_CACHE.get((self.model.in_dim, self.NBUF), [])
                hit = next((i for i, st in enumerate(parked) if st[0]["x"].shape[0] >= rows and st[0]["meta"].shape[1] >= nchunks), None)
                self._stage = parked.pop(hit) if hit is not None else None
            if self._stage is None:
                self._stage = _new_stage(torch, self.model.in_dim, rows, nchunks, self.NBUF)
            if self._finalizer is None:
                import weakref
                self._finalizer = weakref.finalize(self, _park_stage, self._holder)
            self._holder[:] = [(self.model.in_dim, self.NBUF), self._stage]
        if self._copy_stream is None:
            self._copy_stream = torch.cuda.Stream(device=self.model.device)

    PIN_FLOOR = (1024, 64)

    def _regular_caps(self, rows, count, floor, regular_rows):
        rows = max(rows, floor[0]) if rows <= 4096 else max(rows, regular_rows)
        count = max(count, floor[1]) if count <= 64 else max(count, min(self.max_batch_chunks, 8192))
        return rows, count

    def _pinned(self, kind, shape, dtype):
# ... 642 lines not shown
```

x-vector-kaldi-tf_amd/xvector_amd/hiplib.py:

```python
import ctypes
import functools
import os

_HERE = os.path.dirname(os.path.abspath(__file__))
SO_PATH = os.environ.get("XVECTOR_HIP_LIB") or os.path.join(_HERE, "libxvector_hip.so")
ABI_VERSION = 42

_vp, _ci, _cf, _i64, _sz = ctypes.c_void_p, ctypes.c_int, ctypes.c_float, ctypes.c_int64, ctypes.c_size_t
_SIGNATURES = {
    "xv_version": (_ci, []),
    "xv_last_error": (ctypes.c_char_p, []),
    "xv_set_tuning": (_ci, [_ci, _ci]),
    "xv_pack_weights_f32": (_ci, [_vp, _ci, _ci, _vp, _vp]),
    "xv_fold_bn_f32": (_ci, [_vp, _vp, _vp, _vp, _cf, _ci, _vp, _vp, _vp]),
    "xv_fold_shift_taps_f32": (_ci, [_vp, _vp, _vp, _ci, _ci, _ci, _vp, _vp, _vp]),
    "xv_tdnn_layer_f32": (_ci, [_vp, _i64, _ci, _ci, _vp, _vp, _vp, _vp, _ci, _vp, _ci, _ci, _ci, _vp, _vp, _ci, _vp, _vp]),
    "xv_packed_weights_rows_f32_floats": (_sz, [_ci, _ci, _ci, _ci]),
    "xv_pack_weights_rows_f32": (_ci, [_vp, _ci, _ci, _ci, _ci, _vp, _vp]),
    "xv_tdnn_layer_rows_f32": (_ci, [_vp, _i64, _ci, _ci, _vp, _vp, _vp, _vp, _ci, _vp, _ci, _ci, _vp, _vp, _ci, _vp]),
    "xv_toom_supported": (_ci, [_ci, _ci, _ci, _ci]),
    "xv_packed_weights_toom_f32_floats": (_sz, [_ci, _ci, _ci]),
    "xv_pack_weights_toom_f32": (_ci, [_vp, _ci, _ci, _ci, _vp, _vp]),
    "xv_tdnn_layer_toom_f32": (_ci, [_vp, _i64, _ci, _ci, _vp, _vp, _vp, _vp, _ci, _vp, _ci, _ci, _vp, _vp, _ci, _vp]),
    "xv_tdnn_layer_toom_dilated_f32": (_ci, [_vp, _i64, _ci, _ci, _vp, _vp, _vp, _vp, _ci, _vp, _ci, _ci, _ci, _vp, _vp, _ci, _vp]),
    "xv_packed_weights_bf16x3_bytes": (_sz, [_ci, _ci, _ci]),
    "xv_pack_weights_bf16x3": (_ci, [_vp, _ci, _ci, _ci, _vp, _vp]),
    "xv_pack_weights_bf16x3_many": (_ci, [_ci, _vp, _vp, _vp, _vp, _vp, _vp, _vp, _vp]),
    "xv_split_row_bytes": (_sz, [_ci]),
    "xv_split_encode_f32": (_ci, [_vp, _i64, _ci, _ci, _vp, _vp]),
    "xv_split_decode_f32": (_ci, [_vp, _i64, _ci, _vp, _ci, _vp]),
    "xv_tdnn_layer_bf16x3": (_ci, [_vp, _ci, _i64, _ci, _ci, _vp, _vp, _vp, _vp, _ci, _vp, _ci, _ci, _ci, _vp, _vp, _ci, _ci, _vp, _ci, _vp]),
    "xv_tdnn_layer_bf16x3_sums": (_ci, [_vp, _ci, _i64, _ci, _ci, _vp, _vp, _vp, _vp, _ci, _vp, _ci, _ci, _ci, _vp, _vp, _ci, _vp, _ci, _vp, _vp]),
    "xv_tdnn_layer_bf16x3_moments": (_ci, [_vp, _ci, _i64, _ci, _ci, _vp, _vp, _vp, _vp, _ci, _vp, _ci, _ci, _ci, _vp, _vp, _ci, _vp, _ci, _vp, _vp]),
    "xv_block_stats_bytes": (_sz, [_i64, _ci]),
    "xv_tdnn_layer_pool_bf16x3": (_ci, [_vp, _ci, _i64, _ci, _ci, _vp, _vp, _vp, _vp, _ci, _vp, _ci, _ci, _ci, _vp, _vp, _vp]),
    "xv_stats_pool_blocks_f32": (_ci, [_vp, _ci, _vp, _vp, _ci, _cf, _vp, _vp]),
    "xv_tdnn_layer_pool_f32": (_ci, [_vp, _i64, _ci, _ci, _vp, _vp, _vp, _vp, _ci, _vp, _ci, _ci, _ci, _vp, _vp, _vp]),
    "xv_packed_first_bf16x3_bytes": (_sz, [_ci, _ci, _ci]),
    "xv_pack_first_bf16x3": (_ci, [_vp, _ci, _ci, _ci, _vp, _vp]),
    "xv_tdnn_first_bf16x3": (_ci, [_vp, _i64, _ci, _ci, _vp, _vp, _vp, _vp, _ci, _vp, _ci, _ci, _ci, _vp, _vp, _vp]),
    "xv_packed_pair_bf16x3_bytes": (_sz, [_ci, _ci, _ci]),
    "xv_pack_pair_bf16x3": (_ci, [_vp, _vp, _ci, _ci, _ci, _vp, _vp]),
    "xv_tdnn_pair_pool_bf16x3": (_ci, [_vp, _i64, _ci, _ci, _ci, _vp, _vp, _vp, _vp, _vp, _vp, _vp, _vp, _vp, _ci, _vp, _vp, _vp]),
    "xv_packed_weights_f16bf8_bytes": (_sz, [_ci, _ci, _ci]),
    "xv_pack_weights_f16bf8": (_ci, [_vp, _ci, _ci, _ci, _vp, _vp]),
    "xv_split8_encode_f32": (_ci, [_vp, _i64, _ci, _ci, _vp, _vp, _vp]),
    "xv_split8_decode_f32": (_ci, [_vp, _i64, _ci, _vp, _ci, _vp]),
    "xv_tdnn_layer_f16bf8": (_ci, [_vp, _i64, _ci, _vp, _vp, _vp, _vp, _ci, _vp, _ci, _ci, _ci, _vp, _vp, _vp, _ci, _ci, _vp, _vp]),
    "xv_tdnn_layer_pool_f16bf8": (_ci, [_vp, _i64, _ci, _vp, _vp, _vp, _vp, _ci, _vp, _ci, _ci, _ci, _vp, _vp, _vp, _vp]),
    "xv_tdnn_first_f16bf8": (_ci, [_vp, _i64, _ci, _ci, _vp, _vp, _vp, _vp, _ci, _vp, _ci, _ci, _ci, _vp, _vp, _vp, _vp]),
    "xv_packed_pair_f16bf8_bytes": (_sz, [_ci, _ci, _ci]),
    "xv_pack_pair_f16bf8": (_ci, [_vp, _vp, _ci, _ci, _ci, _vp, _vp]),
    "xv_tdnn_pair_pool_f16bf8": (_ci, [_vp, _i64, _ci, _ci, _ci, _vp, _vp, _vp, _vp, _vp, _vp, _vp, _vp, _vp, _ci, _vp, _vp, _vp, _vp]),
    "xv_packed_pair_f16mx6_bytes": (_sz, [_ci, _ci, _ci]),
    "xv_pack_pair_f16mx6": (_ci, [_vp, _vp, _ci, _ci, _ci, _vp, _vp]),
    "xv_tdnn_pair_pool_f16mx6": (_ci, [_vp, _i64, _ci, _ci, _ci, _vp, _vp, _vp, _vp, _vp, _vp, _vp, _vp, _vp, _ci, _vp, _vp, _vp, _vp]),
    "xv_packed_weights_f16mx6_bytes": (_sz, [_ci, _ci, _ci]),
    "xv_pack_weights_f16mx6": (_ci, [_vp, _ci, _ci, _ci, _vp, _vp]),
    "xv_split6_encode_f32": (_ci, [_vp, _i64, _ci, _ci, _vp, _vp, _vp]),
    "xv_split6_decode_f32": (_ci, [_vp, _i64, _ci, _vp, _vp, _ci, _vp]),
    "xv_tdnn_layer_f16mx6": (_ci, [_vp, _i64, _ci, _vp, _vp, _vp, _vp, _ci, _vp, _ci, _ci, _ci, _vp, _vp, _vp, _ci, _ci, _vp, _vp]),
    "xv_fc_bf16x3": (_ci, [_vp, _ci, _ci, _vp, _vp, _vp, _vp, _ci, _vp, _ci, _vp, _vp, _vp]),
    "xv_stats_pool_workspace_bytes": (_sz, [_ci, _ci, _ci, _ci]),
    "xv_stats_pool_f32": (_ci, [_vp, _i64, _ci, _vp, _vp, _ci, _ci, _ci, _cf, _vp, _vp, _vp]),
    "xv_fc_f32": (_ci, [_vp, _ci, _ci, _vp, _vp, _vp, _vp, _ci, _vp, _ci, _vp, _vp, _vp]),
    "xv_fc_splitk_workspace_bytes": (_sz, [_ci, _ci, _ci]),
    "xv_fc_splitk_f32": (_ci, [_vp, _ci, _ci, _vp, _vp, _vp, _vp, _ci, _vp, _ci, _vp, _vp, _vp, _vp]),
    "xv_chunk_average_f32": (_ci, [_vp, _vp, _vp, _ci, _ci, _vp, _vp]),
    "xv_chunk_moments_f32": (_ci, [_vp, _i64, _ci, _vp, _vp, _ci, _ci, _ci, _vp, _vp, _vp]),
    "xv_merge_moments_f32": (_ci, [_vp, _vp, _ci, _ci, _vp, _vp, _vp]),
    "xv_rows_affine_f32": (_ci, [_vp, _ci, _i64, _ci, _vp, _vp, _vp, _vp, _ci, _vp]),
    "xv_rows_affine_split_f32": (_ci, [_vp, _ci, _i64, _ci, _vp, _vp, _vp, _vp, _ci, _vp, _vp]),
    "xv_wgrad_workspace_bytes": (_sz, [_i64, _ci, _ci, _ci]),
    "xv_wgrad_f32": (_ci, [_vp, _ci, _vp, _ci, _i64, _ci, _ci, _ci, _ci, _vp, _vp, _vp]),
    "xv_wgrad_bf16x3": (_ci, [_vp, _ci, _vp, _ci, _i64, _ci, _ci, _ci, _ci, _vp, _vp, _vp]),
    "xv_wgrad_bias_workspace_bytes": (_sz, [_i64, _ci, _ci, _ci]),
    "xv_wgrad_bias_bf16x3": (_ci, [_vp, _ci, _vp, _ci, _i64, _ci, _ci, _ci, _ci, _vp, _vp, _vp, _vp]),
    "xv_col_sums_workspace_bytes": (_sz, [_i64, _ci]),
    "xv_col_sums_f32": (_ci, [_vp, _ci, _vp, _ci, _i64, _ci, _vp, _vp, _vp, _vp]),
    "xv_bn_act_backward_f32": (_ci, [_vp, _vp, _ci, _i64, _ci, _vp, _vp, _vp, _vp, _vp, _cf, _cf, _ci, _cf, _vp, _vp, _vp, _vp, _vp, _vp]),
    "xv_bn_act_backward_split_f32": (_ci, [_vp, _vp, _ci, _i64, _ci, _vp, _vp, _vp, _vp, _vp, _cf, _cf, _ci, _cf, _vp, _vp, _vp, _vp, _vp, _vp, _vp]),
    "xv_bn_act_backward_parts_f32": (_ci, [_vp, _vp, _ci, _i64, _ci, _vp, _vp, _vp, _vp, _cf, _cf, _ci, _cf, _vp, _vp, _vp, _vp, _vp, _vp, _vp]),
    "xv_bn_moments_fold_f32": (_ci, [_vp, _i64, _ci, _cf, _vp, _vp, _cf, _vp, _vp, _vp, _vp, _vp]),
    "xv_col_sums_merge_f32": (_ci, [_vp, _i64, _ci, _vp, _vp, _vp]),
    "xv_pool_bn_act_backward_f32": (_ci, [_vp, _vp, _ci, _ci, _vp, _vp, _ci, _i64, _vp, _vp, _vp, _vp, _vp, _vp, _cf, _cf, _ci, _cf, _vp, _vp, _vp, _vp, _vp, _vp]),
    "xv_bn_small_forward_f32": (_ci, [_vp, _ci, _ci, _ci, _vp, _vp, _cf, _vp, _vp, _vp, _ci, _vp]),
    "xv_bn_small_backward_f32": (_ci, [_vp, _vp, _ci, _ci, _ci, _vp, _vp, _vp, _cf, _ci, _cf, _vp, _vp, _vp, _vp]),
    "xv_pool_backward_f32": (_ci, [_vp, _ci, _ci, _vp, _vp, _ci, _i64, _vp, _vp, _vp, _vp]),
    "xv_softmax_ce_f32": (_ci, [_vp, _vp, _ci, _ci, _vp, _vp, _vp, _vp]),
    "xv_adam_f32": (_ci, [_vp, _vp, _vp, _vp, _i64, _cf, _cf, _cf, _cf, _vp]),
    "xv_axpy_f32": (_ci, [_vp, _vp, _cf, _i64, _vp]),
    "xv_sumsq_workspace_bytes": (_sz, [_i64]),
    "xv_sumsq_f32": (_ci, [_vp, _i64, _vp, _vp, _vp]),
    "xv_dropout_f32": (_ci, [_vp, _ci, _i64, _ci, ctypes.c_uint64, _cf, _vp]),
    "xv_minibatch_layout": (_ci, [_ci, _ci, _ci, _i64, _vp, _vp, _vp, _vp]),
    "xv_pack_minibatch_f32": (_ci, [_vp, _ci, _ci, _ci, _ci, _ci, _ci, _vp, _i64, _vp]),
    "xv_prelu_backward_f32": (_ci, [_vp, _vp, _ci, _i64, _ci, _vp, _vp]),
    "xv_ema_f32": (_ci, [_vp, _vp, _ci, _cf, _vp]),
    "xv_l2_normalize_rows_f32": (_ci, [_vp, _ci, _ci, _ci, _vp, _ci, _vp, _vp]),
    "xv_l2_normalize_backward_f32": (_ci, [_vp, _vp, _vp, _ci, _ci, _vp, _vp]),
    "xv_am_margin_f32": (_ci, [_vp, _vp, _ci, _ci, _cf, _cf, _vp]),
    "xv_attention_scores_f32": (_ci, [_vp, _i64, _i64, _ci, _vp, _vp, _vp, _i64, _vp]),
    "xv_attention_softmax_f32": (_ci, [_vp, _vp, _vp, _ci, _vp, _vp]),
    "xv_attention_pool_workspace_bytes": (_sz, [_ci, _ci, _ci, _ci]),
    "xv_attention_pool_f32": (_ci, [_vp, _i64, _ci, _vp, _vp, _vp, _ci, _ci, _ci, _cf, _vp, _vp, _vp]),
    "xv_attention_pool_backward_f32": (_ci, [_vp, _i64, _ci, _vp, _vp, _vp, _ci, _ci, _vp, _vp, _vp, _i64, _vp, _vp]),
    "xv_attention_softmax_backward_f32": (_ci, [_vp, _vp, _vp, _vp, _ci, _vp, _vp]),
    "xv_attention_scores_backward_f32": (_ci, [_vp, _i64, _vp, _vp, _i64, _ci, _vp, _i64, _vp]),
    "xv_cmn_sliding_scatter_f32": (_ci, [_vp, _ci, _ci, _vp, _vp, _ci, _ci, _ci, _ci, _ci, _vp, _vp, _ci, _vp]),
    "xv_backend_prepare_f32": (_ci, [_vp, _i64, _ci, _ci, _vp, _vp, _vp, _i64, _vp, _ci, _ci, _vp, _vp, _vp, _ci, _vp, _i64, _vp, _vp]),
    "xv_score_matrix_f32": (_ci, [_vp, _vp, _i64, _ci, _ci, _ci, _vp, _vp, _i64, _vp]),
    "xv_score_blocks_f32": (_ci, [_vp, _vp, _i64, _ci, _ci, _vp, _vp, _vp, _ci, _ci, _vp, _i64, _vp, _vp]),
    "xv_score_pairs_f32": (_ci, [_vp, _vp, _i64, _ci, _vp, _vp, _i64, _vp, _vp, _vp]),
    "xv_topk_row_stats_f32": (_ci, [_vp, _i64, _ci, _ci, _ci, _vp, _vp, _vp]),
    "xv_moment_stats_f64": (_ci, [_vp, _i64, _i64, _ci, _vp, _vp, _i64, _vp, _sz, _vp]),
    "xv_moment_stats_workspace_bytes": (_sz, [_i64, _ci]),
    "xv_ahc_average_f64": (_ci, [_vp, _i64, _ci, ctypes.c_double, _ci, _vp, _vp, _vp, _vp, _vp, _vp, _sz, _vp]),
    "xv_ahc_average_workspace_bytes": (_sz, [_ci]),
    "xv_ahc_average_batch_f64": (_ci, [_vp, _i64, _vp, _vp, _vp, _vp, _vp, _ci, _ci, _ci, _vp, _vp, _vp, _vp, _vp, _vp, _vp, _sz, _vp]),
    "xv_ahc_average_batch_workspace_bytes": (_sz, [_ci]),
    "xv_pca_plda_groups_f64": (_ci, [_vp, _i64, _ci, _vp, _ci, _ci, ctypes.c_double, _vp, _vp, _vp, _vp, _vp, _vp, _vp, _vp, _vp, _vp, _vp,
                                     _vp, _vp, _vp, _sz, _vp]),
    "xv_pca_plda_groups_workspace_bytes": (_sz, [_ci, _ci]),
    "xv_backend_prepare_groups_f32": (_ci, [_vp, _i64, _ci, _vp, _ci, _ci, _ci, _vp, _vp, _vp, _vp, _ci, _vp, _i64, _vp, _vp, _vp]),
    "xv_vbx_groups_f64": (_ci, [_vp, _i64, _ci, _vp, _ci, _ci, _vp, _vp, _vp, _ci, _vp, _vp, _vp, ctypes.c_double, ctypes.c_double,
                                ctypes.c_double, ctypes.c_double, _ci, ctypes.c_double, _vp, _vp, _vp, _vp, _vp, _vp, _vp, _vp, _sz, _vp]),
    "xv_vbx_groups_workspace_bytes": (_sz, [_ci, _ci, _ci, _ci]),
    "xv_mfcc_f32": (_ci, [_vp, _ci, _vp, _vp, _vp, _vp, _ci, _i64, _vp, _vp, _vp, _vp, _ci, _ci, _vp, _ci, _vp, _ci, _ci, _ci, _ci,
                          _cf, _cf, _ci, _ci, _ci, _cf, _vp, _i64, _vp, _i64, _vp]),
    "xv_vad_energy_f32": (_ci, [_vp, _i64, _vp, _vp, _ci, _cf, _cf, _ci, _cf, _vp, _vp]),
    "xv_augment_power_f64": (_ci, [_vp, _vp, _vp, _i64, _vp, _vp]),
    "xv_augment_conv_f64": (_ci, [_vp, _vp, _vp, _vp, _i64, _vp, _vp, _vp]),
    "xv_augment_gains_f32": (_ci, [_vp, _ci, _vp, _vp, _vp, _vp, _vp, _vp, _vp, _vp, _vp]),
    "xv_augment_mix_f64": (_ci, [_vp, _vp, _vp, _vp, _vp, _i64, _vp, _vp, _vp]),
    "xv_augment_level_f32": (_ci, [_vp, _ci, _vp, _vp, _vp, _vp]),
    "xv_augment_write": (_ci, [_vp, _vp, _vp, _vp, _i64, _vp, _ci, _vp, _vp]),
    "xv_vad_compact_i32": (_ci, [_vp, _vp, _vp, _ci, _i64, _vp, _vp, _vp]),
    "xv_egs_chunks_f16": (_ci, [_vp, _ci, _ci, _i64, _vp, _vp, _ci, _vp, _vp, _vp, _vp, _vp, _vp, _ci, _ci, _ci, _ci, _ci, _vp, _i64, _vp]),
    "xv_voiced_rank_i32": (_ci, [_vp, _vp, _vp, _ci, _i64, _vp, _vp, _vp]),
    "xv_chunk_row_plan_i32": (_ci, [_vp, _vp, _vp, _vp, _vp, _vp, _ci, _i64, ctypes.c_int32, ctypes.c_int32, _vp, _vp, _vp]),
    "xv_cm_payload_bytes": (_i64, [_ci, _ci]),
    "xv_cm_encode_f32": (_ci, [_vp, _i64, _vp, _vp, _ci, _ci, _vp, _vp, _vp, _vp]),
    "xv_resample_num_output": (_i64, [_i64, _ci, _ci]),
    "xv_resample_f32": (_ci, [_vp, _ci, _vp, _vp, _vp, _vp, _vp, _ci, _vp, _ci, _vp, _vp, _vp, _vp, _i64, _vp, _vp]),
    "xv_wave_decode": (_ci, [_vp, _i64, _vp, _ci, _vp, _i64, _vp, _ci, _vp]),
    "xv_cmn_sliding_gather_f32": (_ci, [_vp, _ci, _ci, _i64, _vp, _vp, _ci, _vp, _vp, _vp, _vp, _vp, _vp, _ci, _ci, _ci, _ci, _ci, _vp,
                                        _ci, _i64, _vp]),
}
SYMBOLS = tuple(_SIGNATURES)

FMT_F32, FMT_SPLIT, FMT_SPLIT8, FMT_SPLIT6 = 0, 1, 2, 3
SPLIT_PAD_BEFORE, SPLIT_PAD_AFTER = 8, 264
TUNE_TILE_ROWS = 1
TUNE_FIRST_TILES = 2
TUNE_FP32_GEMM = 3

ACT_NONE, ACT_RELU, ACT_LRELU, ACT_PRELU = 0, 1, 2, 3

BACKEND_KSTEP = 8
SIDE_PLAIN, SIDE_ENROL, SIDE_TEST, SIDE_COSINE = 0, 1, 2, 3
MOMENT_SLAB = 2048
MOMENT_DIM_MAX = 256
AHC_MAX_N = 32768
AHC_BATCH_MAX_N = 4096
PCA_MAX_DIM = 128
PCA_MAX_SWEEPS = 30
VBX_MAX_SPK = 64
VBX_MAX_ITERS = 100

_lib = None


class XvectorHipError(RuntimeError):
    pass


def load():
    global _lib
    if _lib is not None:
        return _lib
    if not os.path.exists(SO_PATH):
        raise XvectorHipError("HIP extension not built: %s is missing (run `python -c 'import __graft_entry__ as g; "
                              "g.build()'` or `make -C x-vector-kaldi-tf_amd/csrc`)" % SO_PATH)
    import torch
    lib = ctypes.CDLL(SO_PATH)
    for name, (restype, argtypes) in _SIGNATURES.items():
        fn = getattr(lib, name)
        fn.restype, fn.argtypes = restype, argtypes
    if lib.xv_version() != ABI_VERSION:
        raise XvectorHipError("libxvector_hip.so ABI version %d != expected %d" % (lib.xv_version(), ABI_VERSION))
    _lib = lib
    return lib


_GPU_SEEN = []


def require_gpu():
    if _GPU_SEEN:
        return _GPU_SEEN[0]
    lib = load()
    import torch
    if not torch.cuda.is_available():
# ... 240 lines not shown

    def repack(self):
        lib = require_gpu()
        _check(lib.xv_pack_weights_bf16x3_many(self.n, self._w, self._K, self._cin, self._pad, self._cout, self._fwd, self._bwd,
                                               _stream()), "xv_pack_weights_bf16x3_many")


class SplitBuf(object):

    def __init__(self, rows, channels, device, fmt=FMT_SPLIT):
        import torch
        self.rows, self.channels, self.fmt = int(rows), int(channels), int(fmt)
        self.row_bytes = int(load().xv_split_row_bytes(self.channels))
        self.base = torch.zeros((SPLIT_PAD_BEFORE + self.rows + SPLIT_PAD_AFTER) * self.row_bytes, dtype=torch.uint8, device=device)
        self.ptr = self.base.data_ptr() + SPLIT_PAD_BEFORE * self.row_bytes

    def view(self, channels, fmt=None):
        v = object.__new__(SplitBuf)
        v.rows, v.channels, v.base = self.rows, int(channels), self.base
        v.fmt = self.fmt if fmt is None else int(fmt)
        v.row_bytes = int(load().xv_split_row_bytes(v.channels))
        assert v.row_bytes <= self.row_bytes
        v.ptr = self.base.data_ptr() + SPLIT_PAD_BEFORE * v.row_bytes
        return v


def split_encode(x, buf, rows=None, status=None):
    lib = require_gpu()
    _f32(x, "x")
    R = x.shape[0] if rows is None else int(rows)
    assert R <= buf.rows and x.shape[1] == buf.channels
    if buf.fmt in (FMT_SPLIT8, FMT_SPLIT6):
        name = "xv_split8_encode_f32" if buf.fmt == FMT_SPLIT8 else "xv_split6_encode_f32"
        _check(getattr(lib, name)(_ptr(x), R, x.shape[1], x.stride(0), ctypes.c_void_p(buf.ptr), _ptr(status), _stream()), name)
        return
    _check(lib.xv_split_encode_f32(_ptr(x), R, x.shape[1], x.stride(0), ctypes.c_void_p(buf.ptr), _stream()), "xv_split_encode_f32")


def split_decode(buf, rows, out=None, cq=None):
    import torch
    lib = require_gpu()
    if out is None:
        out = torch.empty((rows, buf.channels), dtype=torch.float32, device=buf.base.device)
    if buf.fmt == FMT_SPLIT6:
        assert cq is None or (cq.shape == out.shape and cq.stride(0) == out.stride(0))
        _check(lib.xv_split6_decode_f32(ctypes.c_void_p(buf.ptr), int(rows), buf.channels, _ptr(out), _ptr(cq), out.stride(0), _stream()),
               "xv_split6_decode_f32")
        return out
    assert cq is None
    name = "xv_split8_decode_f32" if buf.fmt == FMT_SPLIT8 else "xv_split_decode_f32"
    _check(getattr(lib, name)(ctypes.c_void_p(buf.ptr), int(rows), buf.channels, _ptr(out), out.stride(0), _stream()), name)
    return out


def tdnn_layer3(x, R, w, bias, scale, shift, act, alpha, dilation, row_valid, y, y_preact=None):
    lib = require_gpu()
    assert isinstance(w, Packed3)
    xp, ldx, xfmt = _operand(x, w.cin, R, "x", (FMT_F32, FMT_SPLIT))
    yp, ldy, yfmt = _operand(y, w.cout, R, "y", (FMT_F32, FMT_SPLIT, None))
    prep, ldpre, _ = _operand(y_preact, w.cout, R, "y_preact", (FMT_F32, None), _DENSE)
    _check(lib.xv_tdnn_layer_bf16x3(xp, xfmt, int(R), w.cin, ldx, _ptr(w.wt), _ptr(bias), _ptr(scale), _ptr(shift), int(act),
                                    _ptr(alpha), w.K, int(dilation), w.cout, _valid(row_valid, R), yp, yfmt, ldy, prep, ldpre,
                                    _stream()), "xv_tdnn_layer_bf16x3")


def col_sums_workspace(rows, c, device):
    return _ws(load().xv_col_sums_workspace_bytes(int(rows), int(c)), device)


def tdnn_layer3_sums(x, R, w, dilation, row_valid, y, sum_r, workspace):
    lib = require_gpu()
    assert isinstance(w, Packed3) and supports_sums(w.cout)
    xp, ldx, xfmt = _operand(x, w.cin, R, "x", (FMT_F32, FMT_SPLIT))
    yp, ldy, _ = _operand(y, w.cout, R, "y", (FMT_F32,))
    sp, lds, _ = _operand(sum_r, w.cout, R, "sum_r", (FMT_F32,))
    _check(lib.xv_tdnn_layer_bf16x3_sums(xp, xfmt, int(R), w.cin, ldx, _ptr(w.wt), None, None, None, ACT_NONE, None, w.K, int(dilation),
                                         w.cout, _valid(row_valid, R), yp, ldy, sp, lds, _ptr(workspace), _stream()),
           "xv_tdnn_layer_bf16x3_sums")


def supports_sums(cout):
    return cout % 8 == 0


def tdnn_layer3_moments(x, R, w, bias, act, alpha, dilation, row_valid, y, y_preact, workspace):
    lib = require_gpu()
    assert isinstance(w, Packed3) and supports_sums(w.cout)
    xp, ldx, xfmt = _operand(x, w.cin, R, "x", (FMT_F32, FMT_SPLIT))
    yp, ldy, _ = _operand(y, w.cout, R, "y", (FMT_F32,))
    prep, ldpre, _ = _operand(y_preact, w.cout, R, "y_preact", (FMT_F32, None), _DENSE)
    _check(lib.xv_tdnn_layer_bf16x3_moments(xp, xfmt, int(R), w.cin, ldx, _ptr(w.wt), _ptr(bias), None, None, int(act), _ptr(alpha), w.K,
                                            int(dilation), w.cout, _valid(row_valid, R), yp, ldy, prep, ldpre, _ptr(workspace),
                                            _stream()), "xv_tdnn_layer_bf16x3_moments")


def bn_moments_fold(workspace, rows, n_frames, gamma, beta, eps, mean, var):
    lib = require_gpu()
    c = gamma.numel()
    scale, shift = _scale_shift(gamma)
    _check(lib.xv_bn_moments_fold_f32(_ptr(workspace), int(rows), c, float(n_frames), _ptr(_f32(gamma, "gamma")), _ptr(_f32(beta, "beta")),
                                      float(eps), _ptr(_f32(mean, "mean")), _ptr(_f32(var, "var")), _ptr(scale), _ptr(shift), _stream()),
           "xv_bn_moments_fold_f32")
    return scale, shift


POOL_BLOCK_ROWS = 8


def block_stats_floats(rows, cout):
    return int(load().xv_block_stats_bytes(int(rows), int(cout))) // 4


def _block_stats(block_stats, R, cout):
    assert _f32(block_stats, "block_stats").numel() >= block_stats_floats(R, cout), "block_stats too small"
    return _ptr(block_stats)


def tdnn_layer_pool(x, R, w, bias, scale, shift, act, alpha, dilation, row_valid, block_stats, K=None):
    lib = require_gpu()
    if not isinstance(w, Packed3):
        _rows2d(x, "x"); _f32(w, "wp")
        cin, cout = x.shape[1], w.shape[0]
        assert K is not None and w.shape[1] == int(K) * cin and x.shape[0] >= R
        _check(lib.xv_tdnn_layer_pool_f32(_ptr(x), int(R), cin, x.stride(0), _ptr(w), _ptr(bias), _ptr(scale), _ptr(shift), int(act),
                                          _ptr(alpha), int(K), int(dilation), cout, _valid(row_valid, R),
                                          _block_stats(block_stats, R, cout), _stream()), "xv_tdnn_layer_pool_f32")
        return
    xp, ldx, fmt = _operand(x, w.cin, R, "x", (FMT_F32, FMT_SPLIT), _DENSE)
    _check(lib.xv_tdnn_layer_pool_bf16x3(xp, fmt, int(R), w.cin, ldx, _ptr(w.wt), _ptr(bias), _ptr(scale), _ptr(shift), int(act),
                                         _ptr(alpha), w.K, int(dilation), w.cout, _valid(row_valid, R),
                                         _block_stats(block_stats, R, w.cout), _stream()), "xv_tdnn_layer_pool_bf16x3")


class PackedFirst(_Packed):
    __slots__ = ("wt", "K", "cin", "cout")


def first_supported(K, cin, cout):
    return int(load().xv_packed_first_bf16x3_bytes(int(K), int(cin), int(cout))) > 0


def pack_first_bf16x3(w3d):
    lib = require_gpu()
    _f32(w3d, "w"); assert w3d.dim() == 3
    return _pack_bytes(lib.xv_packed_first_bf16x3_bytes, lib.xv_pack_first_bf16x3, "xv_pack_first_bf16x3", PackedFirst, (w3d,), w3d.shape,
                       unsupported="K=%d, %d -> %d")


def tdnn_first(x, R, w, bias, scale, shift, act, alpha, dilation, row_valid, y, status=None):
    lib = require_gpu()
    assert isinstance(w, PackedFirst) and isinstance(y, SplitBuf)
    _rows2d(x, "x"); assert x.shape[0] >= R and x.shape[1] >= w.cin
    assert y.channels == w.cout and y.rows >= R
    if y.fmt == FMT_SPLIT8:
        _check(lib.xv_tdnn_first_f16bf8(_ptr(x), int(R), w.cin, x.stride(0), _ptr(w.wt), _ptr(bias), _ptr(scale), _ptr(shift), int(act),
                                        _ptr(alpha), w.K, int(dilation), w.cout, _valid(row_valid, R), ctypes.c_void_p(y.ptr),
                                        _ptr(status), _stream()), "xv_tdnn_first_f16bf8")
        return
    _check(lib.xv_tdnn_first_bf16x3(_ptr(x), int(R), w.cin, x.stride(0), _ptr(w.wt), _ptr(bias), _ptr(scale), _ptr(shift), int(act),
                                    _ptr(alpha), w.K, int(dilation), w.cout, _valid(row_valid, R), ctypes.c_void_p(y.ptr), _stream()),
           "xv_tdnn_first_bf16x3")


class Packed8(_Packed):
    __slots__ = ("wt", "K", "cin", "cout")


def f16bf8_supported(K, dilation):
    span = (int(K) - 1) * int(dilation)
    return int(K) in (1, 3, 5, 7) and (int(K) == 1 or 2 <= span <= 8)


def pack_weights_f16bf8(w3d):
    lib = require_gpu()
    return _pack_bytes(lib.xv_packed_weights_f16bf8_bytes, lib.xv_pack_weights_f16bf8, "xv_pack_weights_f16bf8", Packed8,
                       (_f32(w3d, "w"),), w3d.shape)


def _tap_bias(tapbias, w):
    if tapbias is not None:
        _f32(tapbias, "tapbias")
        assert tuple(tapbias.shape) == (w.K, w.cout), "tapbias must be [K, Cout] = [%d, %d]" % (w.K, w.cout)
    return _ptr(tapbias)


def tdnn_layer8(x, R, w, bias, scale, shift, act, alpha, dilation, row_valid, y, status=None, tapbias=None):
    lib = require_gpu()
    assert isinstance(w, (Packed8, PackedMx6))
    if isinstance(w, PackedMx6):
        return _layer8("xv_tdnn_layer_f16mx6", FMT_SPLIT6, lib, x, R, w, bias, scale, shift, act, alpha, dilation, row_valid, y, status, tapbias)
    _layer8("xv_tdnn_layer_f16bf8", FMT_SPLIT8, lib, x, R, w, bias, scale, shift, act, alpha, dilation, row_valid, y, status, tapbias)


def _layer8(name, xfmt, lib, x, R, w, bias, scale, shift, act, alpha, dilation, row_valid, y, status, tapbias):
    xp = _operand(x, w.cin, R, "x", (xfmt,))[0]
    yp, ldy, yfmt = _operand(y, w.cout, R, "y", (FMT_F32, FMT_SPLIT, FMT_SPLIT8, FMT_SPLIT6))
    _check(getattr(lib, name)(xp, int(R), w.cin, _ptr(w.wt), _ptr(bias), _ptr(scale), _ptr(shift), int(act), _ptr(alpha), w.K,
                              int(dilation), w.cout, _valid(row_valid, R), _tap_bias(tapbias, w), yp, yfmt, ldy, _ptr(status),
                              _stream()), name)


class PackedMx6(_Packed):
    __slots__ = ("wt", "K", "cin", "cout")


def layer_mx6_supported(K, dilation, cin, cout):
    return f16bf8_supported(K, dilation) and int(load().xv_packed_weights_f16mx6_bytes(int(K), int(cin), int(cout))) > 0


def pack_weights_f16mx6(w3d):
    lib = require_gpu()
    return _pack_bytes(lib.xv_packed_weights_f16mx6_bytes, lib.xv_pack_weights_f16mx6, "xv_pack_weights_f16mx6", PackedMx6,
                       (_f32(w3d, "w"),), w3d.shape, unsupported="K = %d, %d -> %d")


def tdnn_layer_mx6(x, R, w, bias, scale, shift, act, alpha, dilation, row_valid, y, status=None, tapbias=None):
    lib = require_gpu()
    assert isinstance(w, PackedMx6)
    _layer8("xv_tdnn_layer_f16mx6", FMT_SPLIT6, lib, x, R, w, bias, scale, shift, act, alpha, dilation, row_valid, y, status, tapbias)


def tdnn_layer_pool8(x, R, w, bias, scale, shift, act, alpha, dilation, row_valid, block_stats, tapbias=None):
    lib = require_gpu()
    assert isinstance(w, Packed8)
    xp = _operand(x, w.cin, R, "x", (FMT_SPLIT8,))[0]
    _check(lib.xv_tdnn_layer_pool_f16bf8(xp, int(R), w.cin, _ptr(w.wt), _ptr(bias), _ptr(scale), _ptr(shift), int(act), _ptr(alpha), w.K,
                                         int(dilation), w.cout, _valid(row_valid, R), _tap_bias(tapbias, w),
                                         _block_stats(block_stats, R, w.cout), _stream()),
           "xv_tdnn_layer_pool_f16bf8")


class PackedPair(_Packed):
    __slots__ = ("wt", "cin", "cmid", "cout")


def pair_supported(cin, cmid, cout):
    return int(load().xv_packed_pair_bf16x3_bytes(int(cin), int(cmid), int(cout))) > 0


def _pack_pair(arith, cls, w1, w2):
    lib = require_gpu()
    _f32(w1, "w1"); _f32(w2, "w2")
    assert w1.dim() == 2 and w2.dim() == 2 and w1.shape[1] == w2.shape[0]
    return _pack_bytes(getattr(lib, "xv_packed_pair_%s_bytes" % arith), getattr(lib, "xv_pack_pair_" + arith), "xv_pack_pair_" + arith,
                       cls, (w1, w2), (w1.shape[0], w1.shape[1], w2.shape[1]), unsupported="%d -> %d -> %d")


def _pair_pool(arith, cls, fmt, x, R, w, p1, p2, act, row_valid, block_stats, *status):
    lib = require_gpu()
    assert isinstance(w, cls)
    xp = _operand(x, w.cin, R, "x", (fmt,))[0]
    name = "xv_tdnn_pair_pool_" + arith
    _check(getattr(lib, name)(xp, int(R), w.cin, w.cmid, w.cout, _ptr(w.wt), _ptr(p1[0]), _ptr(p1[1]), _ptr(p1[2]), _ptr(p1[3]),
                              _ptr(p2[0]), _ptr(p2[1]), _ptr(p2[2]), _ptr(p2[3]), int(act), _valid(row_valid, R),
                              _block_stats(block_stats, R, w.cout), *status, _stream()), name)


def pack_pair_bf16x3(w1, w2):
    return _pack_pair("bf16x3", PackedPair, w1, w2)


class PackedPair8(_Packed):
    __slots__ = ("wt", "cin", "cmid", "cout")


def pair8_supported(cin, cmid, cout):
    return int(load().xv_packed_pair_f16bf8_bytes(int(cin), int(cmid), int(cout))) > 0


def pack_pair_f16bf8(w1, w2):
    return _pack_pair("f16bf8", PackedPair8, w1, w2)


def tdnn_pair_pool8(x, R, w, p1, p2, act, row_valid, block_stats, status=None):
    _pair_pool("f16bf8", PackedPair8, FMT_SPLIT8, x, R, w, p1, p2, act, row_valid, block_stats, _ptr(status))


class PackedPairMx6(_Packed):
    __slots__ = ("wt", "cin", "cmid", "cout")


def pair_mx6_supported(cin, cmid, cout):
    return int(load().xv_packed_pair_f16mx6_bytes(int(cin), int(cmid), int(cout))) > 0


def pack_pair_f16mx6(w1, w2):
    return _pack_pair("f16mx6", PackedPairMx6, w1, w2)


def tdnn_pair_pool_mx6(x, R, w, p1, p2, act, row_valid, block_stats, status=None):
    _pair_pool("f16mx6", PackedPairMx6, FMT_SPLIT8, x, R, w, p1, p2, act, row_valid, block_stats, _ptr(status))


def tdnn_pair_pool(x, R, w, p1, p2, act, row_valid, block_stats):
    _pair_pool("bf16x3", PackedPair, FMT_SPLIT, x, R, w, p1, p2, act, row_valid, block_stats)


def stats_pool_blocks(block_stats, c, row_start, row_len, nchunks, eps, out):
    lib = require_gpu()
    _f32(block_stats, "block_stats"); _f32(out, "out")
    _chunk_tables(row_start, row_len)
    assert out.shape[1] == 2 * c and out.shape[0] >= nchunks
    _check(lib.xv_stats_pool_blocks_f32(_ptr(block_stats), int(c), _ptr(row_start), _ptr(row_len), int(nchunks), float(eps),
                                        _ptr(out), _stream()), "xv_stats_pool_blocks_f32")


def fold_bn(gamma, beta, mean, var, eps):
    lib = require_gpu()
    c = gamma.numel()
    scale, shift = _scale_shift(gamma)
# ... 900 lines not shown
```

Before: 270,400.

## Emit split6 MX-fp6 output from first layer so layer 1 uses mx6 GEMM

Adds a split6 (fp16 high plus MX e2m3-scaled low part) output format to the fused first-layer kernel, so layer 1 can read that format and run the mx6 packed GEMM instead of the bf8 path. The low part is stored in fewer bytes and layer 1 gets cheaper MFMA cross terms, which cuts memory traffic and MFMA work for layer 1. It adds permlane swaps and encode arithmetic to the first-layer epilogue. It also extends the accuracy probe fallback chain with a variant that turns first_mx6 off if the error limit is exceeded.

```diff
diff --git a/include/xvector_hip.h b/include/xvector_hip.h
--- a/include/xvector_hip.h
+++ b/include/xvector_hip.h
@@ -137,6 +137,9 @@
                          const float *bn_shift, int act_kind, const float *act_alpha, int K, int dilation, int cout,
                          const uint8_t *row_valid, const float *tap_bias, void *y, int y_format, int ldy, int32_t *status,
                          void *stream);
+int xv_tdnn_first_f16mx6(const float *x, int64_t R, int cin, int ldx, const void *wt, const float *bias, const float *bn_scale,
+                         const float *bn_shift, int act_kind, const float *act_alpha, int K, int dilation, int cout,
+                         const uint8_t *row_valid, void *y, int32_t *status, void *stream);
 
 int xv_fc_bf16x3(const float *x, int nrows, int in_dim, const void *wt, const float *bias, const float *bn_scale,
                  const float *bn_shift, int act_kind, const float *act_alpha, int out_dim, float *y, float *y_preact, void *stream);
diff --git a/x-vector-kaldi-tf_amd/csrc/xv_first.hip b/x-vector-kaldi-tf_amd/csrc/xv_first.hip
--- a/x-vector-kaldi-tf_amd/csrc/xv_first.hip
+++ b/x-vector-kaldi-tf_amd/csrc/xv_first.hip
@@ -1,5 +1,5 @@
 #include "xv_device.h"
-#include "xv_split8.h"
+#include "xv_split6.h"
 
 namespace {
 
@@ -33,6 +33,8 @@
     int *status;
 };
 
+constexpr int FR_Y3 = 0, FR_Y8 = 1, FR_Y6 = 2;
+
 template <int MODE>
 __device__ __forceinline__ float first_act(float z, float a)
 {
@@ -53,14 +55,21 @@
 
 constexpr int FR_STORE_AUX = 2;
 
-template <int MODE, bool Y8, int NT, bool MASK, bool CLAMP>
+__device__ __forceinline__ void swap_rows16(unsigned &a, unsigned &b)
+{
+    asm("s_nop 1\n\tv_permlane16_swap_b32 %0, %1" : "+v"(a), "+v"(b));
+}
+
+template <int MODE, int YF, int NT, bool MASK, bool CLAMP>
 __device__ __forceinline__ void first_block(const bf16x8 (&xh)[FR_TILES][FR_NKS], const bf16x8 (&xl)[FR_TILES][FR_NKS],
                                             const bf16x8 (&wh0)[FR_NKS], const bf16x8 (&wl0)[FR_NKS], const bf16x8 (&wh1)[FR_NKS],
                                             const bf16x8 (&wl1)[FR_NKS], const f32x4 b0, const f32x4 b1, const f32x4 s0, const f32x4 s1,
-                                            const f32x4 o0, const f32x4 o1, const f32x4 a0, const f32x4 a1, const int (&keepm)[FR_TILES],
+                                            const f32x4 o0, const f32x4 o1, const f32x4 a0r, const f32x4 a1r, const f32x4 *Pa,
+                                            const int (&keepm)[FR_TILES],
                                             const unsigned (&hioff)[FR_TILES], const int slab_off, const __amdgpu_buffer_rsrc_t yrs,
-                                            float &amax)
-{
+                                            const unsigned xoff6, const bool odd, float &amax)
+{
+    constexpr bool Y8 = YF == FR_Y8, Y6 = YF == FR_Y6;
     f32x4 m0[NT], m1[NT];
     auto mfma_tile = [&](int j) {
         m0[j] = b0; m1[j] = b1;
@@ -76,6 +85,11 @@
     };
     auto epilogue = [&](int j) {
         const f32x4 z0 = m0[j], z1 = m1[j];
+        f32x4 a0 = a0r, a1 = a1r;
+        if constexpr (Y6 && MODE != 2) {
+            asm volatile("" ::: "memory");
+            a0 = Pa[0]; a1 = Pa[1];
+        }
         float v[8];
 #pragma unroll
         for (int e = 0; e < 4; e += 2) {
@@ -121,6 +135,46 @@
             vx = (xv_i32x4){__builtin_bit_cast(int, t0), __builtin_bit_cast(int, t1), h0, h1};
             __builtin_amdgcn_raw_buffer_store_b128(vh, yrs, hioff[j], slab_off, FR_STORE_AUX);
             __builtin_amdgcn_raw_buffer_store_b128(vx, yrs, hioff[j] ^ 64u, slab_off, FR_STORE_AUX);
+        } else if constexpr (Y6) {
+            typedef _Float16 f16x2 __attribute__((ext_vector_type(2)));
+            xv_i32x4 vh;
+            xv_f32x16 t16;
+            float t = 0.f, ml = 0.f, mc = 0.f;
+#pragma unroll
+            for (int i = 0; i < 8; i += 2) t = fmaxf(t, fmaxf(fabsf(v[i]), fabsf(v[i + 1])));
+            amax = fmaxf(amax, t);
+#pragma unroll
+            for (int i = 0; i < 8; i += 2) {
+                float ca = v[i], cb = v[i + 1];
+                if constexpr (CLAMP) {
+                    ca = __builtin_amdgcn_fmed3f(ca, -XV_SPLIT8_MAX, XV_SPLIT8_MAX);
+                    cb = __builtin_amdgcn_fmed3f(cb, -XV_SPLIT8_MAX, XV_SPLIT8_MAX);
+                    mc = fmaxf(mc, fmaxf(fabsf(ca), fabsf(cb)));
+                }
+                if constexpr (MASK) {
+                    ca = __builtin_bit_cast(float, __builtin_bit_cast(int, ca) & keepm[j]);
+                    cb = __builtin_bit_cast(float, __builtin_bit_cast(int, cb) & keepm[j]);
+                }
+                const f16x2 h = {(_Float16)ca, (_Float16)cb};
+                vh[i >> 1] = __builtin_bit_cast(int, h);
+                const f32x2 l2 = (f32x2){sub_f16_half<0>(ca, vh[i >> 1]), sub_f16_half<1>(cb, vh[i >> 1])} * XV_SPLIT8_LO_SCALE;
+                ml = fmaxf(ml, fmaxf(fabsf(l2[0]), fabsf(l2[1])));
+                t16[i] = l2[0]; t16[i + 1] = l2[1]; t16[8 + i] = ca; t16[9 + i] = cb;
+            }
+            if constexpr (!CLAMP) mc = t;
+            if constexpr (MASK) mc = __builtin_bit_cast(float, __builtin_bit_cast(int, mc) & keepm[j]);
+            unsigned ma = __builtin_bit_cast(unsigned, fmaxf(mc, ml)), mb = ma;
+            swap_rows16(ma, mb);
+            const int e8m0 = xv_split6_e8m0(fmaxf(__builtin_bit_cast(float, ma), __builtin_bit_cast(float, mb)));
+            const xv_u32x6 dup = xv_cvt_2xpk16_e2m3(t16, t16, __builtin_bit_cast(float, e8m0 << 23));
+            constexpr unsigned EV0 = 0x3f03f03fu, EV1 = 0xf03f03f0u, EV2 = 0x03f03f03u;
+            const unsigned x6[3] = {(dup[0] & EV0) | (dup[3] & ~EV0), (dup[1] & EV1) | (dup[4] & ~EV1), (dup[2] & EV2) | (dup[5] & ~EV2)};
+            unsigned da = x6[0], db = da;
+            swap_rows16(da, db);
+            const xv_i32x4 vx = {(int)(odd ? x6[1] : x6[0]), (int)(odd ? x6[2] : x6[1]), odd ? e8m0 - XV_SPLIT6_LO_EXP : (int)x6[2],
+                                 odd ? 0 : (int)db};
+            __builtin_amdgcn_raw_buffer_store_b128(vh, yrs, hioff[j], slab_off, FR_STORE_AUX);
+            __builtin_amdgcn_raw_buffer_store_b128(vx, yrs, hioff[j] ^ xoff6, slab_off, FR_STORE_AUX);
         } else {
             bf16x8 vh, vl;
 #pragma unroll
@@ -146,7 +200,7 @@
     __builtin_amdgcn_sched_barrier(0);
 }
 
-template <int MODE, bool Y8>
+template <int MODE, int YF>
 __global__ __launch_bounds__(FR_WAVES * 64) void tdnn_first_kernel(const FirstParams p)
 {
     extern __shared__ __attribute__((aligned(16))) char lds[];
@@ -154,6 +208,9 @@
     const int lane = tid & 63;
     const int wave = __builtin_amdgcn_readfirstlane(tid >> 6);
     const int G = lane >> 4, f = lane & 15;
+    const unsigned xoff6 = (unsigned)((G ^ (4 + (G >> 1) + 2 * (G & 1))) << 4);
+    const bool odd = (G & 1) != 0;
+    constexpr bool RANGE = YF != FR_Y3;
     const long tile0 = ((long)blockIdx.x * FR_WAVES + wave) * p.tpw;
     const int left = ((p.K - 1) * p.dil) >> 1;
     const int n_pass = (p.cout + FR_PASS_COLS - 1) / FR_PASS_COLS;
@@ -204,13 +261,15 @@
                 keepm[j] = (in && (!p.valid || p.valid[row])) ? -1 : 0;
                 hioff[j] = in ? (unsigned)lrow * yrow + (unsigned)((G ^ ((int)(row >> 1) & 7)) << 4) : 0x80000000u;
             }
+            int kc = p.kc;
+            if constexpr (YF == FR_Y6) asm volatile("" : "+s"(kc));
 #pragma unroll
             for (int u = 0; u < FR_NKS; ++u) {
                 const int k = 32 * u + 8 * G;
-                const int tap = k / p.kc;
+                const int tap = k / kc;
                 const bool live = tap < p.K;
                 const int tap_off = tap * p.dil - left;
-                const int c0 = k - tap * p.kc;
+                const int c0 = k - tap * kc;
 #pragma unroll
                 for (int j = 0; j < FR_TILES; ++j) {
                     const long r = p.row_base + lrow0 + 16 * j + f + tap_off;
@@ -257,22 +316,22 @@
                 const f32x4 b0 = P4[c4], b1 = P4[c4 + 1], s0 = P4[FR_MAX_COUT / 4 + c4], s1 = P4[FR_MAX_COUT / 4 + c4 + 1],
                             o0 = P4[2 * FR_MAX_COUT / 4 + c4], o1 = P4[2 * FR_MAX_COUT / 4 + c4 + 1];
                 f32x4 a0 = {0.f, 0.f, 0.f, 0.f}, a1 = a0;
-                if constexpr (MODE != 2) { a0 = P4[3 * FR_MAX_COUT / 4 + c4]; a1 = P4[3 * FR_MAX_COUT / 4 + c4 + 1]; }
+                if constexpr (MODE != 2 && YF != FR_Y6) { a0 = P4[3 * FR_MAX_COUT / 4 + c4]; a1 = P4[3 * FR_MAX_COUT / 4 + c4 + 1]; }
                 const int slab_off = (pass * (FR_PASS_COLS / 32) + tp) * SROW;
-                auto run = [&](auto nt, auto mask, auto clamp) {
-                    first_block<MODE, Y8, decltype(nt)::value, decltype(mask)::value, decltype(clamp)::value>(
-                        xh, xl, wh0, wl0, wh1, wl1, b0, b1, s0, s1, o0, o1, a0, a1, keepm, hioff, slab_off, yrs, amax);
+                auto run = [&](auto nt, auto mask, auto clamp) __attribute__((always_inline)) {
+                    first_block<MODE, YF, decltype(nt)::value, decltype(mask)::value, decltype(clamp)::value>(
+                        xh, xl, wh0, wl0, wh1, wl1, b0, b1, s0, s1, o0, o1, a0, a1, P4 + 3 * FR_MAX_COUT / 4 + c4, keepm, hioff, slab_off, yrs, xoff6, odd, amax);
                 };
-                auto run_nt = [&](auto mask, auto clamp) {
+                auto run_nt = [&](auto mask, auto clamp) __attribute__((always_inline)) {
                     if (n_live == 3) run(std::integral_constant<int, 3>{}, mask, clamp);
                     else if (n_live == 2) run(std::integral_constant<int, 2>{}, mask, clamp);
                     else run(std::integral_constant<int, 1>{}, mask, clamp);
                 };
-                if (Y8 && clamping) run_nt(std::true_type{}, std::true_type{});
+                if (RANGE && clamping) run_nt(std::true_type{}, std::true_type{});
                 else {
                     if (group_masked) run_nt(std::true_type{}, std::false_type{});
                     else run_nt(std::false_type{}, std::false_type{});
-                    if (Y8 && __builtin_amdgcn_ballot_w64(!(amax <= XV_SPLIT8_MAX)) != 0) {
+                    if (RANGE && __builtin_amdgcn_ballot_w64(!(amax <= XV_SPLIT8_MAX)) != 0) {
                         clamping = true;
                         run_nt(std::true_type{}, std::true_type{});
                         stores_behind_fetch = -1000;
@@ -284,7 +343,7 @@
         if (++pass == n_pass) pass = 0;
         if (++in_group == n_pass) { in_group = 0; ++group; }
     }
-    if constexpr (Y8)
+    if constexpr (RANGE)
         if (amax > XV_SPLIT8_MAX && p.status) atomicOr(p.status, 1);
 }
 
@@ -341,7 +400,7 @@
 
 static int first_launch(const float *x, int64_t R, int cin, int ldx, const void *wt, const float *bias, const float *bn_scale,
                         const float *bn_shift, int act_kind, const float *act_alpha, int K, int dilation, int cout,
-                        const uint8_t *row_valid, void *y, bool y8, int32_t *status, void *stream)
+                        const uint8_t *row_valid, void *y, int yf, int32_t *status, void *stream)
 {
     if (R <= 0) return 0;
     if (!x || !wt || !y) return fail(XV_ERR_BAD_ARG, "tdnn_first: NULL pointer");
@@ -358,8 +417,9 @@
     p.bias = bias; p.scale = bn_scale; p.shift = bn_shift; p.alpha = act_alpha; p.act = act_kind; p.valid = row_valid;
     p.y = (uint8_t *)y; p.ychunks = cout / 32; p.status = (int *)status;
     typedef void (*kern_t)(const FirstParams);
-    const kern_t kerns[6] = {tdnn_first_kernel<0, false>, tdnn_first_kernel<1, false>, tdnn_first_kernel<2, false>,
-                             tdnn_first_kernel<0, true>,  tdnn_first_kernel<1, true>,  tdnn_first_kernel<2, true>};
+    const kern_t kerns[9] = {tdnn_first_kernel<0, FR_Y3>, tdnn_first_kernel<1, FR_Y3>, tdnn_first_kernel<2, FR_Y3>,
+                             tdnn_first_kernel<0, FR_Y8>, tdnn_first_kernel<1, FR_Y8>, tdnn_first_kernel<2, FR_Y8>,
+                             tdnn_first_kernel<0, FR_Y6>, tdnn_first_kernel<1, FR_Y6>, tdnn_first_kernel<2, FR_Y6>};
     static std::atomic<unsigned long long> lds_done{0};
     if (const int rc = opt_in_dynamic_lds(lds_done, kerns, FR_LDS_BYTES)) return rc;
     const int mode = act_kind == XV_ACT_LRELU ? 1 : act_kind == XV_ACT_RELU ? 2 : 0;
@@ -380,7 +440,7 @@
         p.n_tiles = (p.rows_here + 15) / 16;
         p.tpw = forced > 0 ? forced : (int)((p.n_tiles + waves - 1) / waves);
         const long per_wg = (long)p.tpw * FR_WAVES;
-        hipLaunchKernelGGL(kerns[mode + (y8 ? 3 : 0)], dim3((unsigned)((p.n_tiles + per_wg - 1) / per_wg)), dim3(FR_WAVES * 64), FR_LDS_BYTES,
+        hipLaunchKernelGGL(kerns[mode + 3 * yf], dim3((unsigned)((p.n_tiles + per_wg - 1) / per_wg)), dim3(FR_WAVES * 64), FR_LDS_BYTES,
                            (hipStream_t)stream, p);
     }
     return launch_status();
@@ -390,7 +450,7 @@
                          const float *bn_shift, int act_kind, const float *act_alpha, int K, int dilation, int cout,
                          const uint8_t *row_valid, void *y, void *stream)
 {
-    return first_launch(x, R, cin, ldx, wt, bias, bn_scale, bn_shift, act_kind, act_alpha, K, dilation, cout, row_valid, y, false,
+    return first_launch(x, R, cin, ldx, wt, bias, bn_scale, bn_shift, act_kind, act_alpha, K, dilation, cout, row_valid, y, FR_Y3,
                         nullptr, stream);
 }
 
@@ -398,8 +458,16 @@
                          const float *bn_shift, int act_kind, const float *act_alpha, int K, int dilation, int cout,
                          const uint8_t *row_valid, void *y, int32_t *status, void *stream)
 {
-    return first_launch(x, R, cin, ldx, wt, bias, bn_scale, bn_shift, act_kind, act_alpha, K, dilation, cout, row_valid, y, true,
+    return first_launch(x, R, cin, ldx, wt, bias, bn_scale, bn_shift, act_kind, act_alpha, K, dilation, cout, row_valid, y, FR_Y8,
                         status, stream);
 }
 
-}
+int xv_tdnn_first_f16mx6(const float *x, int64_t R, int cin, int ldx, const void *wt, const float *bias, const float *bn_scale,
+                         const float *bn_shift, int act_kind, const float *act_alpha, int K, int dilation, int cout,
+                         const uint8_t *row_valid, void *y, int32_t *status, void *stream)
+{
+    return first_launch(x, R, cin, ldx, wt, bias, bn_scale, bn_shift, act_kind, act_alpha, K, dilation, cout, row_valid, y, FR_Y6,
+                        status, stream);
+}
+
+}
diff --git a/x-vector-kaldi-tf_amd/csrc/xv_kernels.hip b/x-vector-kaldi-tf_amd/csrc/xv_kernels.hip
--- a/x-vector-kaldi-tf_amd/csrc/xv_kernels.hip
+++ b/x-vector-kaldi-tf_amd/csrc/xv_kernels.hip
@@ -786,7 +786,7 @@
 void xv_internal_gemm8_tile_rows(int value);
 void xv_internal_first_tiles(int tiles);
 
-int xv_version(void) { return 42; }
+int xv_version(void) { return 43; }
 
 int xv_set_tuning(int key, int value)
 {
diff --git a/x-vector-kaldi-tf_amd/local/tf/models.py b/x-vector-kaldi-tf_amd/local/tf/models.py
--- a/x-vector-kaldi-tf_amd/local/tf/models.py
+++ b/x-vector-kaldi-tf_amd/local/tf/models.py
@@ -178,7 +178,8 @@
         elif known is not None:
             self.device_model = engine.DeviceModel(w, meta["topology"], _device(), self.embedding_index, known["selected"],
                                                    fold_shift=False if known.get("fold_shift") is False else None,
-                                                   layer_mx6=False if known.get("layer_mx6") is False else None)
+                                                   layer_mx6=False if known.get("layer_mx6") is False else None,
+                                                   first_mx6=False if known.get("first_mx6") is False else None)
             self.device_model.selection = dict(known, cached=True)
             self._model_key = key
         else:
diff --git a/x-vector-kaldi-tf_amd/xvector_amd/engine.py b/x-vector-kaldi-tf_amd/xvector_amd/engine.py
--- a/x-vector-kaldi-tf_amd/xvector_amd/engine.py
+++ b/x-vector-kaldi-tf_amd/xvector_amd/engine.py
@@ -237,7 +237,7 @@
     POOL_SPLIT_ROWS = 512
 
     def __init__(self, weights, topo, device="cuda:0", embedding_index=0, precision="bf16x3", fused_pool=None, pair_kernel=None,
-                 first_kernel=None, fold_shift=None, layer_mx6=None):
+                 first_kernel=None, fold_shift=None, layer_mx6=None, first_mx6=None):
         import torch
         hiplib.require_gpu()
         assert precision in ("fp32", "fp32tc", "bf16x3", "f16bf8")
@@ -340,6 +340,14 @@
             self.layer_mx6 = bool(self.mx6_layers)
             assert not (layer_mx6 and not self.layer_mx6), \
                 "layer_mx6=True needs an f16bf8 model with a K in {3,5,7} layer (Cin % 64 == 0, Cout % 256 == 0) behind another one"
+            self.first_mx6 = False
+            if self.f16bf8 and (first_mx6 is None or first_mx6) and (n - 2 if self.pair is not None else n - 1) > 1:
+                L1 = self.layers[1]
+                if hiplib.layer_mx6_supported(L1["K"], L1["dil"], L1["cin"], L1["cout"]):
+                    L1["wp6"] = hiplib.pack_weights_f16mx6(self._wdev(weights, "frame_level_info_layer-1/w:0"))
+                    self.first_mx6 = True
+            assert not (first_mx6 and not self.first_mx6), \
+                "first_mx6=True needs an f16bf8 model whose layer 1 has K in {3,5,7}, Cin % 64 == 0, Cout % 256 == 0 and is not part of the pair kernel"
             can_fold = self.f16bf8 and self.act == tp.ACT_RELU and all(L["cout"] % 8 == 0 for L in self.layers[1:] if L["K"] > 1)
             self.fold_shift = can_fold and (fold_shift is None or bool(fold_shift))
             assert not (fold_shift and not self.fold_shift), \
@@ -536,7 +544,7 @@
         L = self.layers[0]
         stop = n - 2 if self.pair is not None else n - 1
         pair_fmt = S8 if self.pair8 is not None else S3
-        h = bufs[0].view(L["cout"], pair_fmt if (self.pair is not None and stop == 1) else S8)
+        h = bufs[0].view(L["cout"], pair_fmt if (self.pair is not None and stop == 1) else S6 if self.first_mx6 else S8)
         mark("start")
         if self.first is not None:
             hiplib.tdnn_first(x, R, self.first, *ep(0), L["dil"], row_valid, h, status)
@@ -544,13 +552,14 @@
         else:
             y32 = self._l0_rows[:R]
             hiplib.tdnn_layer(x, L["wp"], *ep(0), L["K"], L["dil"], row_valid, y32, rows=R)
-            hiplib.split_encode(y32, h, rows=R, status=status if h.fmt == S8 else None)
+            hiplib.split_encode(y32, h, rows=R, status=status if h.fmt in (S8, S6) else None)
             mark("layer 0: tdnn_gemm_bf16x3_kernel + split encode")
         for i in range(1, stop):
             L = self.layers[i]
             y = bufs[i & 1].view(L["cout"], pair_fmt if (self.pair is not None and i == stop - 1) else
                                  S6 if i + 1 in self.mx6_layers else S8)
-            hiplib.tdnn_layer8(h, R, L["wp6" if i in self.mx6_layers else "wp8"], *ep(i), L["dil"], row_valid, y, status, tapbias=taps(i))
+            mx6 = i in self.mx6_layers or (i == 1 and self.first_mx6)
+            hiplib.tdnn_layer8(h, R, L["wp6" if mx6 else "wp8"], *ep(i), L["dil"], row_valid, y, status, tapbias=taps(i))
             mark("layer %d: tdnn_gemm_f16bf8 (K=%d, %d -> %d)" % (i, L["K"], L["cin"], L["cout"]))
             h = y
         if self.pair is not None:
@@ -660,10 +669,11 @@
     return float(np.nan_to_num(r, nan=np.inf).max()) if len(r) else 0.0
 
 
-def select_model(weights, topo, device="cuda:0", embedding_index=0, precision="f16bf8", probe=None, fold_shift=None, layer_mx6=None):
+def select_model(weights, topo, device="cuda:0", embedding_index=0, precision="f16bf8", probe=None, fold_shift=None, layer_mx6=None,
+                 first_mx6=None):
     if probe is None:
         probe = os.environ.get("XVECTOR_ACCURACY_PROBE", "1") != "0"
-    model = DeviceModel(weights, topo, device, embedding_index, precision, fold_shift=fold_shift, layer_mx6=layer_mx6)
+    model = DeviceModel(weights, topo, device, embedding_index, precision, fold_shift=fold_shift, layer_mx6=layer_mx6, first_mx6=first_mx6)
     sel = dict(requested=precision, selected=model.arithmetic, probed=False)
     model.selection = sel
     if not probe or not model.f16bf8:
@@ -675,13 +685,13 @@
     twin = model.fallback()
     ref = twin.probe_vectors(batch)
     err = _max_rel_l2(got, ref)
-    sel.update(probed=True, layer_mx6=model.layer_mx6, f16bf8_vs_bf16x3=err, f16bf8_limit=PROBE_LIMIT_F16BF8, probe_left_fp16_range=clamped,
+    sel.update(probed=True, layer_mx6=model.layer_mx6, first_mx6=model.first_mx6, f16bf8_vs_bf16x3=err, f16bf8_limit=PROBE_LIMIT_F16BF8, probe_left_fp16_range=clamped,
                probe_frames=int(np.sum(batch[2])))
     if err <= PROBE_LIMIT_F16BF8 and not clamped:
         return model
     last, last_err = model, err
     if model.fold_shift and fold_shift is None:
-        plain = DeviceModel(weights, topo, device, embedding_index, precision, fold_shift=False, layer_mx6=layer_mx6)
+        plain = DeviceModel(weights, topo, device, embedding_index, precision, fold_shift=False, layer_mx6=layer_mx6, first_mx6=first_mx6)
         got = plain.probe_vectors(batch)
         clamped2 = int(plain.status.item()) != 0
         plain.status.zero_()
@@ -692,8 +702,21 @@
             plain.selection = sel
             return plain
         last, last_err = plain, err2
+    if last.first_mx6 and first_mx6 is None:
+        l1 = DeviceModel(weights, topo, device, embedding_index, precision, fold_shift=last.fold_shift, layer_mx6=layer_mx6, first_mx6=False)
+        got = l1.probe_vectors(batch)
+        clamped1 = int(l1.status.item()) != 0
+        l1.status.zero_()
+        err_l1 = _max_rel_l2(got, ref)
+        sel.update(first_mx6_f16bf8_vs_bf16x3=last_err, f16bf8_vs_bf16x3=err_l1, probe_left_fp16_range=clamped1, first_mx6=False)
+        if err_l1 <= PROBE_LIMIT_F16BF8 and not clamped1:
+            l1._fallback = twin
+            l1.selection = sel
+            return l1
+        last, last_err = l1, err_l1
     if last.layer_mx6 and layer_mx6 is None:
-        bf8 = DeviceModel(weights, topo, device, embedding_index, precision, fold_shift=last.fold_shift, layer_mx6=False)
+        bf8 = DeviceModel(weights, topo, device, embedding_index, precision, fold_shift=last.fold_shift, layer_mx6=False,
+                          first_mx6=False if first_mx6 is None else first_mx6)
         got = bf8.probe_vectors(batch)
         clamped3 = int(bf8.status.item()) != 0
         bf8.status.zero_()
diff --git a/x-vector-kaldi-tf_amd/xvector_amd/hiplib.py b/x-vector-kaldi-tf_amd/xvector_amd/hiplib.py
--- a/x-vector-kaldi-tf_amd/xvector_amd/hiplib.py
+++ b/x-vector-kaldi-tf_amd/xvector_amd/hiplib.py
@@ -4,7 +4,7 @@
 
 _HERE = os.path.dirname(os.path.abspath(__file__))
 SO_PATH = os.environ.get("XVECTOR_HIP_LIB") or os.path.join(_HERE, "libxvector_hip.so")
-ABI_VERSION = 42
+ABI_VERSION = 43
 
 _vp, _ci, _cf, _i64, _sz = ctypes.c_void_p, ctypes.c_int, ctypes.c_float, ctypes.c_int64, ctypes.c_size_t
 _SIGNATURES = {
@@ -49,6 +49,7 @@
     "xv_tdnn_layer_f16bf8": (_ci, [_vp, _i64, _ci, _vp, _vp, _vp, _vp, _ci, _vp, _ci, _ci, _ci, _vp, _vp, _vp, _ci, _ci, _vp, _vp]),
     "xv_tdnn_layer_pool_f16bf8": (_ci, [_vp, _i64, _ci, _vp, _vp, _vp, _vp, _ci, _vp, _ci, _ci, _ci, _vp, _vp, _vp, _vp]),
     "xv_tdnn_first_f16bf8": (_ci, [_vp, _i64, _ci, _ci, _vp, _vp, _vp, _vp, _ci, _vp, _ci, _ci, _ci, _vp, _vp, _vp, _vp]),
+    "xv_tdnn_first_f16mx6": (_ci, [_vp, _i64, _ci, _ci, _vp, _vp, _vp, _vp, _ci, _vp, _ci, _ci, _ci, _vp, _vp, _vp, _vp]),
     "xv_packed_pair_f16bf8_bytes": (_sz, [_ci, _ci, _ci]),
     "xv_pack_pair_f16bf8": (_ci, [_vp, _vp, _ci, _ci, _ci, _vp, _vp]),
     "xv_tdnn_pair_pool_f16bf8": (_ci, [_vp, _i64, _ci, _ci, _ci, _vp, _vp, _vp, _vp, _vp, _vp, _vp, _vp, _vp, _ci, _vp, _vp, _vp, _vp]),
@@ -595,10 +596,11 @@
     assert isinstance(w, PackedFirst) and isinstance(y, SplitBuf)
     _rows2d(x, "x"); assert x.shape[0] >= R and x.shape[1] >= w.cin
     assert y.channels == w.cout and y.rows >= R
-    if y.fmt == FMT_SPLIT8:
-        _check(lib.xv_tdnn_first_f16bf8(_ptr(x), int(R), w.cin, x.stride(0), _ptr(w.wt), _ptr(bias), _ptr(scale), _ptr(shift), int(act),
-                                        _ptr(alpha), w.K, int(dilation), w.cout, _valid(row_valid, R), ctypes.c_void_p(y.ptr),
-                                        _ptr(status), _stream()), "xv_tdnn_first_f16bf8")
+    if y.fmt in (FMT_SPLIT8, FMT_SPLIT6):
+        name = "xv_tdnn_first_f16bf8" if y.fmt == FMT_SPLIT8 else "xv_tdnn_first_f16mx6"
+        _check(getattr(lib, name)(_ptr(x), int(R), w.cin, x.stride(0), _ptr(w.wt), _ptr(bias), _ptr(scale), _ptr(shift), int(act),
+                                  _ptr(alpha), w.K, int(dilation), w.cout, _valid(row_valid, R), ctypes.c_void_p(y.ptr),
+                                  _ptr(status), _stream()), name)
         return
     _check(lib.xv_tdnn_first_bf16x3(_ptr(x), int(R), w.cin, x.stride(0), _ptr(w.wt), _ptr(bias), _ptr(scale), _ptr(shift), int(act),
                                     _ptr(alpha), w.K, int(dilation), w.cout, _valid(row_valid, R), ctypes.c_void_p(y.ptr), _stream()),
```

Measured after the change: 278,500, median of 6. 1.03x the previous value.
